# Gardlin/PCR-CG

Measured on AMD Instinct MI355X. Metric: fragment-pairs/s KPFCNN+GCN fwd, 30k-pt pairs, higher is better.
Workload: dtype f32

## Files before the change

### include/pcrcg.h

```cpp
#ifndef PCRCG_H
#define PCRCG_H

#include <stddef.h>
#include <stdint.h>

#ifdef __cplusplus
extern "C" {
#endif

#define PCRCG_OK 0
#define PCRCG_EBADARG (-1)
#define PCRCG_EWORKSPACE (-2)
#define PCRCG_ELAUNCH (-3)
#define PCRCG_ECAPACITY (-4)

#define PCRCG_KPOINTS 15

const char* pcrcg_last_error(void);
#define PCRCG_ABI_VERSION 4
int pcrcg_abi_version(void);

int pcrcg_debug_set(const char* spec);
int pcrcg_debug_release(void);

// ... 47 lines not shown
    int forest_ns, forest_nb;
} pcrcg_reorder_job;
size_t pcrcg_kdforest_ws_bytes(int ns, int nb);
int pcrcg_kdforest_build(const float* sup, int ns, const int* slen, int nb, void* forest, size_t forest_bytes,
                         void* stream);
int pcrcg_radius_reorder(const float* q, int nq, const int* qlen, int nbq, const float* sup, int ns, int nb,
                         const void* forest, int cloud0, float radius, const int* rows, int nrows, const int* count,
                         int max_count, int cols, int64_t* idx, int* status, void* stream);
int pcrcg_radius_reorder_jobs(const pcrcg_reorder_job* jobs, int njobs, const float* sup, int ns, int nb,
                              const void* forest, int* status, void* stream);

size_t pcrcg_kpconv_ws_bytes(int ns);
int pcrcg_kpconv_aggregate(const float* q_pts, int nq, const float* s_pts, int ns, const int64_t* idx,
                           int h, int ld_idx, const float* x, int cin, const float* kp, float extent,
                           float* wf, float* inv_n, void* ws, size_t ws_bytes, void* stream);
int pcrcg_kpconv_c1_layer(const float* q_pts, int nq, const float* s_pts, int ns, const int64_t* idx, int h, int ld_idx,
                          const float* x, const float* kp, float extent, const float* wt, int cout, float* out, int ld_out,
                          float* inv_n, void* sums, void* ws, size_t ws_bytes, void* stream);
int pcrcg_kpconv_aggregate_bf16(const float* q_pts, int nq, const float* s_pts, int ns, const int64_t* idx, int h,
                                int ld_idx, const float* x, int cin, const float* kp, float extent, void* x_bf16,
                                void* wf_bf16, float* inv_n, void* ws, size_t ws_bytes, void* stream);

int pcrcg_kpconv_aggregate_ex(const float* q_pts, int nq, const float* s_pts, int ns, const int64_t* idx, int h,
                              int ld_idx, const float* x, int cin, const float* kp, float extent,
                              const float* offset_features, int ld_off, int influence, int closest, int modulated,
                              float* wf, float* inv_n, float* min_d2, void* ws, size_t ws_bytes, void* stream);

int pcrcg_query_walk(const float* points, int n, int* walk, int* key, void* stream);
int pcrcg_kpconv_aggregate_walk(const float* q_pts, int nq, const float* s_pts, int ns, const int64_t* idx,
                                int h, int ld_idx, const float* x, int cin, const float* kp, float extent,
                                float* wf, float* inv_n, void* ws, size_t ws_bytes, const int* walk, void* stream);
int pcrcg_kpconv_aggregate_bf16_walk(const float* q_pts, int nq, const float* s_pts, int ns, const int64_t* idx, int h,
                                     int ld_idx, const float* x, int cin, const float* kp, float extent, void* x_bf16,
                                     void* wf_bf16, float* inv_n, void* ws, size_t ws_bytes, const int* walk, void* stream);
int pcrcg_gather_max_walk(const float* x, int ns, int c, const int64_t* idx, int nq, int h, int ld_idx,
                          float* out, const int* walk, void* stream);

void pcrcg_profile_kpconv(int enable);
int pcrcg_profile_kpconv_read(float* ms, int* nq, int* h, int* cin, int* cout, int* kind, int cap);

int pcrcg_gemm_f32(const float* a, int lda, const float* b, int ldb, int trans_b, float* c, int ldc, int m,
                   int n, int k, const float* row_scale, const float* bias, void* stream);
size_t pcrcg_gemm_colstats_bytes(int m, int n);
int pcrcg_gemm_f32_colstats(const float* a, int lda, const float* b, int ldb, int trans_b, float* c, int ldc,
                            int m, int n, int k, const float* row_scale, const float* bias, void* colstats,
                            size_t colstats_bytes, int* h_chunks, void* stream);
int pcrcg_gemm_bf16a_f32_colstats(const void* a_bf16, int lda, const float* b, int ldb, float* c, int ldc, int m, int n,
                                  int k, const float* row_scale, const float* bias, void* colstats,
                                  size_t colstats_bytes, int* h_chunks, void* stream);

int pcrcg_gemm_f32_fused(const float* a, int lda, const int64_t* idx, int ld_idx, int ns, const float* zero_row,
                         const void* a_sums, double a_count, float a_eps, float a_slope, const float* b, int ldb,
                         const float* bias, float* c, int ldc, int m, int n, int k, int accumulate, void* stream);

void pcrcg_gemm_set_mode(int mode);
int pcrcg_gemm_get_mode(void);
int pcrcg_gemm_redo_counts(unsigned long long* out2, int reset);
void pcrcg_thread_shares_gpu(int on);

int pcrcg_gather_max(const float* x, int ns, int c, const int64_t* idx, int nq, int h, int ld_idx,
                     float* out, void* stream);
int pcrcg_gather_first(const float* x, int ns, int c, const int64_t* idx, int nq, int ld_idx, float* out,
                       int ld_out, void* stream);
int pcrcg_gather_first_multi(const float* const* x, const int* ns, const int64_t* const* idx, const int* nq, const int* ld_idx,
                             float* const* out, int count, int c, int ld_x, int ld_out, void* stream);
size_t pcrcg_instnorm_ws_bytes(int c);
int pcrcg_instnorm_stats_from_partials(const void* partials, int chunks, int c, double count, float eps,
                                       float* stats, void* stream);
int pcrcg_instnorm_stats(const float* x, int n, int c, int ldx, float eps, float* stats, void* ws,
                         size_t ws_bytes, void* stream);
int pcrcg_instnorm_apply(const float* x, int n, int c, int ldx, const float* stats, const float* res,
                         int ldr, const float* res_stats, float slope, float* y, int ldy, void* stream);
int pcrcg_instnorm_colsums(const float* x, int n, int c, int ldx, void* sums, void* stream);
int pcrcg_instnorm_apply_sums(const float* x, int n, int c, int ldx, const void* sums, double count, float eps,
                              const float* res, int ldr, const void* res_sums, float slope, float* y, int ldy,
                              void* stream);

int pcrcg_fill2d(float* dst, int ld, int rows, int cols, float value, void* stream);
int pcrcg_inject_image_features(const float* fmap, int c, int h, int w, const float* valid, const int64_t* inds2d,
                                const int64_t* inds3d, int n, long row_offset, long n_rows, float* x, int ldx,
                                void* stream);

typedef struct pcrcg_image_frame {
    const float* fmap;
    const float* depth;
    const float* valid;
    float world2camera[16];
    float intrinsics[16];
    float thresh;
    int h, w;
    int depth_h, depth_w;
    int target;
} pcrcg_image_frame;

size_t pcrcg_project_depth_ws_bytes(int n);
int pcrcg_project_depth(const float* points, int n, const float* depth, int h, int w, const float* h_world2camera,
                        const float* h_intrinsics, float thresh, int64_t* inds2d, int64_t* inds3d, int* k, void* ws,
                        size_t ws_bytes, void* stream);
int pcrcg_inject_frames(const float* points, long n_points, long len_src, const pcrcg_image_frame* h_frames, int n_frames,
                        int c, float* x, int ldx, void* stream);
int pcrcg_superglue_valid_maps(const float* keypoints0, int n0, const float* keypoints1, int n1, const int64_t* matches,
                               const float* confidence, int window, int map_w, int map_h, float* src_valid, float* tgt_valid,
                               void* stream);

int pcrcg_knn(const float* coords, int n, int k, int* idx, void* stream);
size_t pcrcg_edgeconv_ws_bytes(int c);
int pcrcg_edgeconv_reduce(const float* ctr, int ld_ctr, const float* nbr, int ld_nbr, const int* idx,
                          int n, int k, int c, float eps, float* emax, int ld_emax, float* stats,
                          void* ws, size_t ws_bytes, void* stream);
int pcrcg_edgeconv_reduce_sums(const float* ctr, int ld_ctr, const float* nbr, int ld_nbr, const int* idx, int n, int k,
                               int c, float* emax, int ld_emax, void* sums, void* stream);
int pcrcg_softmax_rows(float* x, int rows, int cols, int ld, float scale, void* stream);
int pcrcg_attention_supported(int d);
int pcrcg_attention(const float* q, int ldq, const float* k, int ldk, const float* v, int ldv, float* out, int ldo, int n,
                    int ms, int heads, int d, float scale, void* stream);
int pcrcg_softmax_matvec(const float* x, int rows, int cols, int ld, float scale, const float* vec, int ldv, float* y,
                         int ldy, void* stream);

// ... 202 lines not shown
```

### pcrcg_amd/_lib.py

```python
import ctypes
import os

_HERE = os.path.dirname(os.path.abspath(__file__))
LIB_PATH = os.path.join(_HERE, "libpcrcg_hip.so")


def lib_identity():
    import hashlib
    with open(LIB_PATH, "rb") as f:
        return LIB_PATH, hashlib.sha256(f.read()).hexdigest()[:16]

ABI_VERSION = 4

c_int, c_float, c_void_p, c_size_t = ctypes.c_int, ctypes.c_float, ctypes.c_void_p, ctypes.c_size_t

SIGNATURES = {
    "pcrcg_last_error": (ctypes.c_char_p, []),
    "pcrcg_abi_version": (c_int, []),
    "pcrcg_debug_set": (c_int, [ctypes.c_char_p]),
    "pcrcg_check_status": (c_int, [c_void_p, c_void_p]),
    "pcrcg_grid_subsample_ws_bytes": (c_size_t, [c_int, c_int]),
    "pcrcg_grid_subsample_batch": (c_int, [c_void_p, c_int, c_void_p, c_int, c_float, c_int, c_void_p, c_void_p,
                                           c_void_p, c_void_p, c_size_t, c_void_p]),
    "pcrcg_grid_subsample_ex_ws_bytes": (c_size_t, [c_int, c_int, c_int, c_int]),
    "pcrcg_grid_subsample_batch_ex": (c_int, [c_void_p, c_int, c_void_p, c_int, c_float, c_int, c_void_p, c_int, c_int,
                                              c_void_p, c_int, c_void_p, c_void_p, c_void_p, c_void_p, c_void_p, c_void_p,
                                              c_size_t, c_void_p]),
    "pcrcg_umap_order_ws_bytes": (c_size_t, [c_int]),
    "pcrcg_umap_order": (c_int, [c_void_p, c_int, c_void_p, c_void_p, c_size_t, c_void_p]),
    "pcrcg_cellgrid_ws_bytes": (c_size_t, [c_int, c_int]),
    "pcrcg_cellgrid_build": (c_int, [c_void_p, c_int, c_void_p, c_int, c_float, c_void_p, c_size_t, c_void_p]),
    "pcrcg_radius_query": (c_int, [c_void_p, c_int, c_void_p, c_int, c_void_p, c_int, c_float, c_void_p, c_int,
                                   c_void_p, c_void_p, c_void_p, c_void_p, c_void_p]),
    "pcrcg_radius_query_ex": (c_int, [c_void_p, c_int, c_void_p, c_int, c_void_p, c_int, c_float, c_void_p, c_int,
                                      c_void_p, c_void_p, c_void_p, c_void_p, c_void_p, c_void_p, c_void_p]),
    "pcrcg_radius_query_groups": (c_int, [c_void_p, c_int, c_void_p, c_int, c_void_p, c_int, c_int, c_float, c_void_p, c_int,
                                          c_void_p, c_void_p, c_void_p, c_void_p, c_void_p, c_void_p, c_void_p]),
    "pcrcg_radius_query_cells": (c_int, [c_void_p, c_void_p, c_int, c_void_p, c_void_p, c_int, c_void_p, c_int, c_int, c_float,
                                         c_int, c_void_p, c_void_p, c_void_p, c_void_p, c_void_p, c_void_p, c_void_p]),
    "pcrcg_kdforest_ws_bytes": (c_size_t, [c_int, c_int]),
    "pcrcg_kdforest_build": (c_int, [c_void_p, c_int, c_void_p, c_int, c_void_p, c_size_t, c_void_p]),
    "pcrcg_radius_reorder": (c_int, [c_void_p, c_int, c_void_p, c_int, c_void_p, c_int, c_int, c_void_p, c_int,
                                     c_float, c_void_p, c_int, c_void_p, c_int, c_int, c_void_p, c_void_p, c_void_p]),
    "pcrcg_radius_reorder_jobs": (c_int, [c_void_p, c_int, c_void_p, c_int, c_int, c_void_p, c_void_p, c_void_p]),
    "pcrcg_radius_neighbors_ws_bytes": (c_size_t, [c_int, c_int]),
    "pcrcg_radius_neighbors_batch": (c_int, [c_void_p, c_int, c_void_p, c_int, c_void_p, c_void_p, c_int, c_float,
                                             c_int, c_void_p, c_void_p, c_void_p, c_void_p, c_void_p, c_size_t,
                                             c_void_p]),
    "pcrcg_kpconv_ws_bytes": (c_size_t, [c_int]),
    "pcrcg_kpconv_aggregate": (c_int, [c_void_p, c_int, c_void_p, c_int, c_void_p, c_int, c_int, c_void_p, c_int,
                                       c_void_p, c_float, c_void_p, c_void_p, c_void_p, c_size_t, c_void_p]),
    "pcrcg_kpconv_c1_layer": (c_int, [c_void_p, c_int, c_void_p, c_int, c_void_p, c_int, c_int, c_void_p, c_void_p, c_float,
                                      c_void_p, c_int, c_void_p, c_int, c_void_p, c_void_p, c_void_p, c_size_t, c_void_p]),
    "pcrcg_kpconv_aggregate_bf16": (c_int, [c_void_p, c_int, c_void_p, c_int, c_void_p, c_int, c_int, c_void_p, c_int,
                                            c_void_p, c_float, c_void_p, c_void_p, c_void_p, c_void_p, c_size_t,
                                            c_void_p]),
    "pcrcg_kpconv_aggregate_ex": (c_int, [c_void_p, c_int, c_void_p, c_int, c_void_p, c_int, c_int, c_void_p, c_int,
                                          c_void_p, c_float, c_void_p, c_int, c_int, c_int, c_int, c_void_p, c_void_p,
                                          c_void_p, c_void_p, c_size_t, c_void_p]),
    "pcrcg_query_walk": (c_int, [c_void_p, c_int, c_void_p, c_void_p, c_void_p]),
    "pcrcg_kpconv_aggregate_walk": (c_int, [c_void_p, c_int, c_void_p, c_int, c_void_p, c_int, c_int, c_void_p, c_int,
                                            c_void_p, c_float, c_void_p, c_void_p, c_void_p, c_size_t, c_void_p, c_void_p]),
    "pcrcg_kpconv_aggregate_bf16_walk": (c_int, [c_void_p, c_int, c_void_p, c_int, c_void_p, c_int, c_int, c_void_p, c_int,
                                                 c_void_p, c_float, c_void_p, c_void_p, c_void_p, c_void_p, c_size_t,
                                                 c_void_p, c_void_p]),
    "pcrcg_gather_max_walk": (c_int, [c_void_p, c_int, c_int, c_void_p, c_int, c_int, c_int, c_void_p, c_void_p, c_void_p]),
    "pcrcg_profile_kpconv": (None, [c_int]),
    "pcrcg_profile_kpconv_read": (c_int, [c_void_p, c_void_p, c_void_p, c_void_p, c_void_p, c_void_p, c_int]),
    "pcrcg_gemm_f32": (c_int, [c_void_p, c_int, c_void_p, c_int, c_int, c_void_p, c_int, c_int, c_int, c_int,
                               c_void_p, c_void_p, c_void_p]),
    "pcrcg_gemm_colstats_bytes": (c_size_t, [c_int, c_int]),
    "pcrcg_gemm_f32_colstats": (c_int, [c_void_p, c_int, c_void_p, c_int, c_int, c_void_p, c_int, c_int, c_int, c_int,
                                        c_void_p, c_void_p, c_void_p, c_size_t, c_void_p, c_void_p]),
    "pcrcg_gemm_bf16a_f32_colstats": (c_int, [c_void_p, c_int, c_void_p, c_int, c_void_p, c_int, c_int, c_int, c_int,
                                              c_void_p, c_void_p, c_void_p, c_size_t, c_void_p, c_void_p]),
    "pcrcg_gemm_f32_fused": (c_int, [c_void_p, c_int, c_void_p, c_int, c_int, c_void_p, c_void_p, ctypes.c_double, c_float,
                                     c_float, c_void_p, c_int, c_void_p, c_void_p, c_int, c_int, c_int, c_int, c_int, c_void_p]),
    "pcrcg_gemm_set_mode": (None, [c_int]),
    "pcrcg_gemm_get_mode": (c_int, []),
    "pcrcg_gemm_redo_counts": (c_int, [c_void_p, c_int]),
    "pcrcg_instnorm_stats_from_partials": (c_int, [c_void_p, c_int, c_int, ctypes.c_double, c_float, c_void_p,
                                                   c_void_p]),
    "pcrcg_gather_max": (c_int, [c_void_p, c_int, c_int, c_void_p, c_int, c_int, c_int, c_void_p, c_void_p]),
    "pcrcg_gather_first": (c_int, [c_void_p, c_int, c_int, c_void_p, c_int, c_int, c_void_p, c_int, c_void_p]),
    "pcrcg_gather_first_multi": (c_int, [c_void_p, c_void_p, c_void_p, c_void_p, c_void_p, c_void_p, c_int, c_int, c_int, c_int,
                                         c_void_p]),
    "pcrcg_instnorm_ws_bytes": (c_size_t, [c_int]),
    "pcrcg_instnorm_stats": (c_int, [c_void_p, c_int, c_int, c_int, c_float, c_void_p, c_void_p, c_size_t, c_void_p]),
    "pcrcg_instnorm_apply": (c_int, [c_void_p, c_int, c_int, c_int, c_void_p, c_void_p, c_int, c_void_p, c_float,
                                     c_void_p, c_int, c_void_p]),
    "pcrcg_instnorm_colsums": (c_int, [c_void_p, c_int, c_int, c_int, c_void_p, c_void_p]),
    "pcrcg_instnorm_apply_sums": (c_int, [c_void_p, c_int, c_int, c_int, c_void_p, ctypes.c_double, c_float, c_void_p, c_int,
                                          c_void_p, c_float, c_void_p, c_int, c_void_p]),
    "pcrcg_fill2d": (c_int, [c_void_p, c_int, c_int, c_int, c_float, c_void_p]),
    "pcrcg_inject_image_features": (c_int, [c_void_p, c_int, c_int, c_int, c_void_p, c_void_p, c_void_p, c_int, ctypes.c_long,
                                            ctypes.c_long, c_void_p, c_int, c_void_p]),
    "pcrcg_project_depth_ws_bytes": (c_size_t, [c_int]),
    "pcrcg_project_depth": (c_int, [c_void_p, c_int, c_void_p, c_int, c_int, c_void_p, c_void_p, c_float, c_void_p, c_void_p,
                                    c_void_p, c_void_p, c_size_t, c_void_p]),
    "pcrcg_inject_frames": (c_int, [c_void_p, ctypes.c_long, ctypes.c_long, c_void_p, c_int, c_int, c_void_p, c_int, c_void_p]),
    "pcrcg_superglue_valid_maps": (c_int, [c_void_p, c_int, c_void_p, c_int, c_void_p, c_void_p, c_int, c_int, c_int, c_void_p,
                                           c_void_p, c_void_p]),
    "pcrcg_knn": (c_int, [c_void_p, c_int, c_int, c_void_p, c_void_p]),
    "pcrcg_edgeconv_ws_bytes": (c_size_t, [c_int]),
    "pcrcg_edgeconv_reduce": (c_int, [c_void_p, c_int, c_void_p, c_int, c_void_p, c_int, c_int, c_int, c_float,
                                      c_void_p, c_int, c_void_p, c_void_p, c_size_t, c_void_p]),
    "pcrcg_edgeconv_reduce_sums": (c_int, [c_void_p, c_int, c_void_p, c_int, c_void_p, c_int, c_int, c_int, c_void_p, c_int,
                                           c_void_p, c_void_p]),
    "pcrcg_softmax_rows": (c_int, [c_void_p, c_int, c_int, c_int, c_float, c_void_p]),
    "pcrcg_attention_supported": (c_int, [c_int]),
    "pcrcg_attention": (c_int, [c_void_p, c_int, c_void_p, c_int, c_void_p, c_int, c_void_p, c_int, c_int, c_int, c_int,
                                c_int, c_float, c_void_p]),
    "pcrcg_softmax_matvec": (c_int, [c_void_p, c_int, c_int, c_int, c_float, c_void_p, c_int, c_void_p, c_int, c_void_p]),
    "pcrcg_copy2d": (c_int, [c_void_p, c_int, c_void_p, c_int, c_int, c_int, c_void_p]),
    "pcrcg_add": (c_int, [c_void_p, c_void_p, c_void_p, ctypes.c_long, c_void_p]),
    "pcrcg_l2norm_rows": (c_int, [c_void_p, c_int, c_void_p, c_int, c_int, c_int, c_void_p]),
    "pcrcg_sigmoid_scores": (c_int, [c_void_p, c_int, c_void_p, c_int, c_void_p]),
    "pcrcg_kpfcnn_ws_bytes": (c_size_t, [c_void_p, c_void_p]),
    "pcrcg_kpfcnn_group_ws_bytes": (c_size_t, [c_void_p, c_void_p, c_int]),
    "pcrcg_kpfcnn_forward_group": (c_int, [c_void_p, c_void_p, c_void_p, c_int, c_void_p, c_size_t, c_void_p]),
    "pcrcg_kpfcnn_forward": (c_int, [c_void_p, c_void_p, c_void_p, c_void_p, c_size_t, c_void_p]),
    "pcrcg_pyramid_ws_bytes": (c_size_t, [c_int, c_int, c_void_p]),
    "pcrcg_pyramid_build": (c_int, [c_void_p, c_int, c_void_p, c_int, c_void_p, c_void_p, c_size_t, c_void_p, c_void_p,
                                    c_void_p, c_void_p, c_void_p, c_void_p]),
    "pcrcg_pyramid_build_parts": (c_int, [c_void_p, c_void_p, c_void_p, c_void_p, c_int, c_void_p, c_void_p, c_size_t, c_void_p,
                                          c_void_p, c_void_p, c_void_p, c_void_p, c_void_p]),
    "pcrcg_pyramid_restore_run": (c_int, [c_void_p, c_void_p, c_void_p]),
    "pcrcg_debug_release": (c_int, []),
    "pcrcg_stream_pipe_classes": (c_int, [c_void_p, c_int, c_void_p, c_void_p]),
    "pcrcg_thread_shares_gpu": (None, [c_int]),
    "pcrcg_stream_create": (c_int, [c_void_p, c_int]),
    "pcrcg_stream_destroy": (c_int, [c_void_p]),
    "pcrcg_ransac_ws_bytes": (c_size_t, [c_int, c_int, c_int, c_int]),
    "pcrcg_feature_match": (c_int, [c_void_p, c_int, c_int, c_void_p, c_int, c_int, c_int, c_int, c_void_p, c_void_p,
                                    c_void_p, c_size_t, c_void_p]),
    "pcrcg_ransac": (c_int, [c_void_p, c_int, c_void_p, c_int, c_void_p, c_void_p, c_int, c_void_p, c_int, ctypes.c_double,
                             ctypes.c_double, c_int, c_int, c_int, ctypes.c_uint64, c_void_p, c_void_p, c_void_p, c_void_p,
# ... 141 lines not shown
```

### pcrcg_amd/csrc/common.h

```cpp
#pragma once
#include <hip/hip_runtime.h>

#include <cstdarg>
#include <cstdint>
#include <cstdio>
#include <map>
#include <mutex>

#include "pcrcg.h"

namespace pcrcg {

void set_error(const char* fmt, ...);

inline hipStream_t as_stream(void* s) { return reinterpret_cast<hipStream_t>(s); }

struct Carver {
    char* base;
    size_t cap;
    size_t off = 0;
    Carver(void* ws, size_t bytes) : base(static_cast<char*>(ws)), cap(bytes) {}
    template <typename T>
    T* take(size_t count) {
        size_t bytes = (count * sizeof(T) + 255) & ~size_t(255);
// ... 10 lines not shown

constexpr int kWave = 64;

bool instnorm_pack_ok(int c, int ldx, int ldy);
int instnorm_apply_pack(const float* x, int n, int c, int ldx, const float* stats, const double* sums, double count, float eps,
                        float slope, float* y, int ldy, const float* s_pts, float4* pk, hipStream_t st);
size_t colstats_ws_bytes(int c);
int colstats_finalize(const double* partial, int nchunks, int c, double count, float eps, float* stats,
                      hipStream_t st);
int colstats_chunks();
float4* kpconv_pk_ptr(void* ws, size_t ws_bytes, int ns);

class StreamScratch {
public:
    explicit StreamScratch(bool cleared = false);
    void* get(hipStream_t st, size_t bytes, size_t slack = 0);
    void release();
private:
    struct Buf { void* p = nullptr; size_t bytes = 0; };
    const bool cleared_;
    std::mutex mu_;
    std::map<hipStream_t, Buf> bufs_;
};

int kpconv_pack(const float* x, int ns, int cin, const float* s_pts, void* ws, size_t ws_bytes, hipStream_t st,
                unsigned short* x_bf16 = nullptr);
int kpconv_aggregate_rows(const float* q_pts, int nq, const float* s_pts, int ns, const int64_t* idx, int h, int ld_idx,
                          const float* x, int cin, const float* kp, float extent, float* wf, float* inv_n, void* ws,
                          size_t ws_bytes, hipStream_t st, bool pack, bool stream_out, int c1_ld = 0,
                          const int* walk = nullptr);
bool kpconv_c1_fused_ok(int cout, const float* wt);
int kpconv_c1_fused(const float* q_pts, int nq, const float* s_pts, int ns, const int64_t* idx, int h, int ld_idx, const float* x,
                    const float* kp, float extent, const float* wt, int cout, float* y, int ld_y, float* inv_n, double* sums,
                    void* ws, size_t ws_bytes, hipStream_t st, bool pack);
int kpconv_aggregate_bf16(const float* q_pts, int nq, const float* s_pts, int ns, const int64_t* idx, int h, int ld_idx,
                          const float* x, unsigned short* x_bf16, int cin, const float* kp, float extent,
                          unsigned short* wf_bf16, float* inv_n, void* ws, size_t ws_bytes, hipStream_t st,
                          const int* walk = nullptr);

int query_walk_multi(const float* const* pts, const int* n, int* const* walk, int* const* key, int count, hipStream_t st);

struct NormJob {
    const float* x; const double* sums; const float* res; const double* res_sums; float* y;
    const float* s_pts; float4* pk;
    int n; double count;
    float* stats_out = nullptr;
};
int instnorm_apply_sums_multi(const NormJob* jobs, int count, int c, int ldx, float eps, int ldr, float slope, int ldy, bool pack,
                              hipStream_t st);
bool instnorm_sums_ok(int c, int ldx, int ldy, int ldr = 0);

struct GatherJob { const float* x; const int64_t* idx; float* out; int ns, nq, h, ld_idx; const int* walk = nullptr; };
int gather_max_multi(const GatherJob* jobs, int count, int c, hipStream_t st);
struct FirstJob { const float* x; const int64_t* idx; float* out; int ns, nq, ld_idx; };
int gather_first_multi(const FirstJob* jobs, int count, int c, int ld_x, int ld_out, hipStream_t st);
int heads_multi(const float* const* x, const int* rows, int count, int ld, int fd, float* const* feats, float* const* s_ov,
                float* const* s_sal, hipStream_t st);
int copy2d_multi(const float* const* src, float* const* dst, const int* rows, int count, int ld_src, int ld_dst, int cols,
                 hipStream_t st);
int instnorm_colsums_multi(const float* const* x, double* const* sums, const int* n, int count, int c, int ldx, hipStream_t st);

struct EdgeCloud {
    const float* ctr; const float* nbr; const int* idx; float* emax; double* sums; int n, k;
};
bool edgeconv_rows_ok(const EdgeCloud* cl, int count, int ld_ctr, int ld_nbr, int ld_emax, int c);
int edgeconv_rows_multi(const EdgeCloud* cl, int count, int ld_ctr, int ld_nbr, int ld_emax, int c, bool atomic, int* nchunks_out,
                        hipStream_t st);

struct AttnCloud { const float* q; const float* k; const float* v; float* out; int n, ms; };
bool attention_mfma_ok(const AttnCloud* cl, int count, int ldq, int ldk, int ldv, int d);
int attention_mfma_multi(const AttnCloud* cl, int count, int ldq, int ldk, int ldv, int ldo, int heads, int d, float scale,
                         hipStream_t st);
bool attention_bwd_mfma_ok(int n, int ms, int d, int ldq, int ldk, int ldv, int ld_do);
int attention_bwd_mfma(const float* q, int ldq, const float* k, int ldk, const float* v, int ldv, const float* o, int ldo,
                       const float* d_o, int ld_do, float* dq, int ld_dq, float* dk, int ld_dk, float* dv, int ld_dv, int n, int ms,
                       int heads, int d, float scale, hipStream_t st);

struct DebugOpts {
    int stat_sums = 1;
    int stat_sums_rows = 1 << 30;
    int att_mfma = 1;
    int radius_blocks = 0;
    int kd_blocks = 0;
    int att_tq = 16;
    int kd_spin_limit = 0;
    int gemm_log = 0;
    int x6_tile = -1, x6_splitk = 0, x6_t1 = 1, x6_t2 = 1, x6_order = -1, x6_big = 0, x6_h2 = 1;
    int train_side_stream = 1;
    int gemm_tile = -1, gemm_splitk = 0, gemm_split_target = 768;
    int deterministic = 0;
    int bwd_mfma = 1;
    int walk = 1;
};
const DebugOpts& debug_opts();

struct KpProfScope {
    hipStream_t st;
    hipEvent_t a, b;
    int nq, h, cin, cout, kind;
    bool on;
    KpProfScope(hipStream_t s, int nq, int h, int cin, int cout, int kind);
    ~KpProfScope();
};

}

#define PCRCG_CHECK_ARG(cond)                                                        \
    do {                                                                             \
        if (!(cond)) {                                                               \
            pcrcg::set_error("%s: bad argument: %s", __func__, #cond);               \
            return PCRCG_EBADARG;                                                    \
        }                                                                            \
    } while (0)

#define PCRCG_CHECK_WS(carver)                                                                     \
    do {                                                                                           \
        if (!(carver).ok()) {                                                                      \
            pcrcg::set_error("%s: workspace too small (%zu needed, %zu given)", __func__,          \
                             (carver).off, (carver).cap);                                          \
            return PCRCG_EWORKSPACE;                                                               \
        }                                                                                          \
    } while (0)

#define PCRCG_CHECK_HIP(expr)                                                                  \
    do {                                                                                       \
        hipError_t e_ = (expr);                                                                \
        if (e_ != hipSuccess) {                                                                \
            pcrcg::set_error("%s: %s failed: %s", __func__, #expr, hipGetErrorString(e_));     \
            return PCRCG_ELAUNCH;                                                              \
        }                                                                                      \
    } while (0)

#define PCRCG_CHECK_LAUNCH() PCRCG_CHECK_HIP(hipGetLastError())

namespace pcrcg {
inline hipError_t grant_max_dyn_lds(const void* kern) {
    hipFuncAttributes at;
    hipError_t e = hipFuncGetAttributes(&at, kern);
    if (e != hipSuccess) return e;
    const int cap = 160 * 1024 - (int)at.sharedSizeBytes;
    return hipFuncSetAttribute(kern, hipFuncAttributeMaxDynamicSharedMemorySize, cap);
}
}
#define PCRCG_GRANT_LDS(kern)                                                                                   \
    do {                                                                                                        \
// ... 12 lines not shown
```

### pcrcg_amd/csrc/gemm.h

```cpp
#pragma once
#include "common.h"

namespace pcrcg {

struct GemmExtra {
    const long long* a_idx = nullptr;
    int a_idx_ld = 0, a_ns = 0;
    const float* a_zero = nullptr;
    bool accumulate = false;
    const double* a_sums = nullptr;
    double a_count = 0.0;
    float a_eps = 1e-5f, a_slope = 1.0f;
    int grad_operand = 0;
};

struct GemmPair {
    const float* a = nullptr;
    float* c = nullptr;
    int m = 0;
    const float* row_scale = nullptr;
    void* colstats = nullptr;
    int* h_chunks = nullptr;
    bool c_zeroed = false;
    const long long* a_idx = nullptr;
    int a_ns = 0;
    const double* a_sums = nullptr;
    double a_count = 0.0;
};
struct GemmGroup {
    int n = 0;
    GemmPair p[3];
};

enum class GemmA { row_f32, kmajor_f32, row_bf16 };
enum class GemmB { nk, kn };

struct GemmCall {
    const void* a = nullptr;
    const float* b = nullptr;
    float* c = nullptr;
    int lda = 0, ldb = 0, ldc = 0;
    int m = 0, n = 0, k = 0;
    GemmA a_form = GemmA::row_f32;
    GemmB b_form = GemmB::nk;
    const float* row_scale = nullptr;
    const float* bias = nullptr;
    void* colstats = nullptr;
    size_t colstats_bytes = 0;
    int* h_chunks = nullptr;
    bool colstats_sums = false;
    bool c_zeroed = false;
    const GemmExtra* ex = nullptr;
    const GemmGroup* grp = nullptr;
    hipStream_t st = nullptr;
};

int gemm_run(const GemmCall& g);
bool gemm_split_terms_on();
bool gemm_bt_accumulates(int m, int n, int k, long m_total = 0);

int gemm_x6_dispatch(const GemmCall& g);
int gemm_x6_splits(int m, int n, int k, long m_total);
int gemm_x6_redo_counts(unsigned long long* out, int reset);
bool gemm_x6_shared();
void gemm_x6_set_shared(int on);

}
```

### pcrcg_amd/csrc/gemm.hip

```cpp
#include <cstdlib>

#include <atomic>

#include "gemm.h"
#include "pcrcg_train.h"

namespace pcrcg {
namespace {

typedef float f32x16 __attribute__((ext_vector_type(16)));
template <int BM, int BN, bool TRANS_A, bool TRANS_B, int BK>
constexpr int stage_floats() {
    return (TRANS_A ? BK * (BM + 4) : BM * (BK + 4)) + (TRANS_B ? BN * (BK + 4) : BK * (BN + 4));
}

template <int BM, int BN, int WAVES_M, int WAVES_N, bool TRANS_A, bool TRANS_B, int BK>
__global__ void __launch_bounds__(256) k_gemm_f32(const float* __restrict__ A, int lda, const float* __restrict__ B,
                                                   int ldb, float* __restrict__ C, int ldc, int M, int N, int Kdim,
                                                   const float* __restrict__ row_scale, const float* __restrict__ bias,
                                                   int k_per_split, int vec_a, int vec_b, int atomic_out,
                                                   double* __restrict__ colp, int colp_chunks) {
    static_assert(WAVES_M * WAVES_N == 4, "4 wavefronts per block");
    constexpr int WM = BM / WAVES_M, WN = BN / WAVES_N;
    constexpr int TM = WM / 32, TN = WN / 32;
// ... 302 lines not shown
        return (long)((m + tiles[t].bm - 1) / tiles[t].bm) * ((n + tiles[t].bn - 1) / tiles[t].bn);
    };
    int pick = debug_opts().gemm_tile;
    if (pick < 0 || pick > 3) pick = (n > 64 && ntiles(0) >= 1024) ? 0 : 3;
    if (trans_a) pick = 3;
    const int BM = tiles[pick].bm, BN = tiles[pick].bn;
    const int gx = (n + BN - 1) / BN, gy = (m + BM - 1) / BM;
    int splits = 1;
    const int ktiles = (k + BK - 1) / BK;
    const int split_target = debug_opts().gemm_split_target;
    const int max_splits = trans_a ? 256 : 32;
    while ((long)gx * gy * splits < split_target && k / (2 * splits) >= 192 && splits < max_splits) splits *= 2;
    if (debug_opts().gemm_splitk > 0) splits = debug_opts().gemm_splitk;
    p.k_per_split = ((ktiles + splits - 1) / splits) * BK;
    if (p.k_per_split < BK) p.k_per_split = BK;
    splits = k > 0 ? (k + p.k_per_split - 1) / p.k_per_split : 1;
    if (splits < 1) splits = 1;
    p.atomic_out = splits > 1;
    if (p.atomic_out) {
        if (g.ldc == n) PCRCG_CHECK_HIP(hipMemsetAsync(g.c, 0, (size_t)m * n * sizeof(float), g.st));
        else PCRCG_CHECK_HIP(hipMemset2DAsync(g.c, (size_t)g.ldc * sizeof(float), 0, (size_t)n * sizeof(float), m, g.st));
    }
    const dim3 grid(gx, gy, splits);
    const bool want_partials = g.colstats && g.h_chunks && !g.colstats_sums;
    if (debug_opts().gemm_log != 0)
        fprintf(stderr, "pcrcg_gemm m=%d n=%d k=%d lda=%d ldb=%d ldc=%d tb=%d grid=%dx%dx%d rs=%d bias=%d stats=%d\n", m, n, k,
                g.lda, g.ldb, g.ldc, (int)trans_b, gx, gy, splits, g.row_scale != nullptr, g.bias != nullptr,
                g.colstats != nullptr && !g.colstats_sums);
    if (want_partials && !p.atomic_out) {
        const int chunks = gy * (pick == 1 ? 4 : 2);
        if (carve_bytes(2 * (size_t)n * chunks, sizeof(double)) <= g.colstats_bytes) {
            p.colp = static_cast<double*>(g.colstats);
            p.colp_chunks = *g.h_chunks = chunks;
        }
    }
    if (trans_a)
        return trans_b ? launch_f32<64, 64, 2, 2, true, true>(p, grid, g.st) : launch_f32<64, 64, 2, 2, true, false>(p, grid, g.st);
    if (pick == 0) return launch_f32_tile<128, 128, 2, 2>(trans_b, p, grid, g.st);
    if (pick == 1) return launch_f32_tile<128, 64, 4, 1>(trans_b, p, grid, g.st);
    if (pick == 2) return launch_f32_tile<64, 128, 2, 2>(trans_b, p, grid, g.st);
    return launch_f32_tile<64, 64, 2, 2>(trans_b, p, grid, g.st);
}

}

bool gemm_split_terms_on() { return gemm_mode() == 1; }

bool gemm_bt_accumulates(int m, int n, int k, long m_total) { return gemm_split_terms_on() && gemm_x6_splits(m, n, k, m_total) > 1; }

int gemm_run(const GemmCall& g) {
    if (g.h_chunks) *g.h_chunks = 0;
    const bool trans_a = g.a_form == GemmA::kmajor_f32, b_kn = g.b_form == GemmB::kn, bf16 = g.a_form == GemmA::row_bf16;
    const bool grouped = g.grp && g.grp->n != 0;
    const bool x6_form = g.ex || grouped || bf16;
    PCRCG_CHECK_ARG(g.m >= 0 && g.n >= 0 && g.k >= 0);
    const bool ld_ok = (trans_a ? g.lda >= g.m : g.lda >= g.k) && (b_kn ? g.ldb >= g.n : g.ldb >= g.k) && g.ldc >= g.n;
    if (x6_form) PCRCG_CHECK_ARG(g.k >= 1 && ld_ok && !(trans_a && !b_kn));
    if (grouped) PCRCG_CHECK_ARG(g.m >= 1 && g.n >= 1);
    if (bf16) PCRCG_CHECK_ARG(g.k % 32 == 0 && g.lda % 8 == 0);
    if (g.m == 0 || g.n == 0) return PCRCG_OK;
    PCRCG_CHECK_ARG(g.a && g.b && g.c);
    PCRCG_CHECK_ARG(ld_ok);
    if (bf16) {
        PCRCG_CHECK_ARG((reinterpret_cast<uintptr_t>(g.a) & 15) == 0 && g.ldb % 4 == 0 && (reinterpret_cast<uintptr_t>(g.b) & 15) == 0);
        return gemm_x6_dispatch(g);
    }
    if (x6_form) PCRCG_CHECK_ARG(gemm_split_terms_on());
    if (gemm_split_terms_on() && !(trans_a && !b_kn)) return gemm_x6_dispatch(g);
    return gemm_f32_dispatch(g);
}

}

using namespace pcrcg;

extern "C" void pcrcg_gemm_set_mode(int mode) { g_gemm_mode.store(mode != 0, std::memory_order_relaxed); }
extern "C" int pcrcg_gemm_get_mode(void) { return gemm_mode(); }
extern "C" void pcrcg_thread_shares_gpu(int on) { gemm_x6_set_shared(on); }
extern "C" int pcrcg_gemm_redo_counts(unsigned long long* out2, int reset) { return gemm_x6_redo_counts(out2, reset); }

extern "C" size_t pcrcg_gemm_colstats_bytes(int m, int n) {
    const size_t chunks = (size_t)((m > 0 ? m : 1) + 31) / 32 + 4;
    return carve_bytes(2 * (size_t)(n > 0 ? n : 1) * chunks, sizeof(double));
}

static GemmCall plain_call(const void* a, int lda, int trans_a, const float* b, int ldb, int trans_b, float* c, int ldc, int m,
                           int n, int k, const float* row_scale, const float* bias, void* stream) {
    GemmCall g;
    g.a = a; g.lda = lda; g.b = b; g.ldb = ldb; g.c = c; g.ldc = ldc;
    g.m = m; g.n = n; g.k = k;
    g.a_form = trans_a ? GemmA::kmajor_f32 : GemmA::row_f32;
    g.b_form = trans_b ? GemmB::nk : GemmB::kn;
    g.row_scale = row_scale; g.bias = bias;
    g.st = as_stream(stream);
    return g;
}

extern "C" int pcrcg_gemm_f32(const float* a, int lda, const float* b, int ldb, int trans_b, float* c, int ldc,
                              int m, int n, int k, const float* row_scale, const float* bias, void* stream) {
    return gemm_run(plain_call(a, lda, 0, b, ldb, trans_b, c, ldc, m, n, k, row_scale, bias, stream));
}

extern "C" int pcrcg_gemm_f32_colstats(const float* a, int lda, const float* b, int ldb, int trans_b, float* c,
                                       int ldc, int m, int n, int k, const float* row_scale, const float* bias,
                                       void* colstats, size_t colstats_bytes, int* h_chunks, void* stream) {
    GemmCall g = plain_call(a, lda, 0, b, ldb, trans_b, c, ldc, m, n, k, row_scale, bias, stream);
    g.colstats = colstats; g.colstats_bytes = colstats_bytes; g.h_chunks = h_chunks;
    return gemm_run(g);
}

extern "C" int pcrcg_gemm_bf16a_f32_colstats(const void* a_bf16, int lda, const float* b, int ldb, float* c, int ldc, int m,
                                             int n, int k, const float* row_scale, const float* bias, void* colstats,
                                             size_t colstats_bytes, int* h_chunks, void* stream) {
    GemmCall g = plain_call(a_bf16, lda, 0, b, ldb, 1, c, ldc, m, n, k, row_scale, bias, stream);
    g.a_form = GemmA::row_bf16;
    g.colstats = colstats; g.colstats_bytes = colstats_bytes; g.h_chunks = h_chunks;
    return gemm_run(g);
}

extern "C" int pcrcg_gemm_f32_fused(const float* a, int lda, const int64_t* idx, int ld_idx, int ns, const float* zero_row,
                                    const void* a_sums, double a_count, float a_eps, float a_slope, const float* b, int ldb,
                                    const float* bias, float* c, int ldc, int m, int n, int k, int accumulate, void* stream) {
    PCRCG_CHECK_ARG(!idx || (ld_idx >= 1 && ns >= 0 && zero_row));
    PCRCG_CHECK_ARG(!a_sums || a_count >= 1.0);
    if (!gemm_split_terms_on()) {
        set_error("pcrcg_gemm_f32_fused: only the split-bf16 arithmetic (pcrcg_gemm_set_mode(1)) implements it");
        return PCRCG_EBADARG;
    }
    GemmExtra ex;
    ex.a_idx = reinterpret_cast<const long long*>(idx);
    ex.a_idx_ld = ld_idx;
    ex.a_ns = ns;
    ex.a_zero = zero_row;
    ex.accumulate = accumulate != 0;
    ex.a_sums = static_cast<const double*>(a_sums);
    ex.a_count = a_count;
    ex.a_eps = a_eps;
    ex.a_slope = a_slope;
    GemmCall g = plain_call(a, lda, 0, b, ldb, 1, c, ldc, m, n, k, nullptr, bias, stream);
    g.ex = &ex;
    return gemm_run(g);
}

extern "C" int pcrcg_gemm_f32_ex(const float* a, int lda, int trans_a, const float* b, int ldb, int trans_b, float* c,
                                 int ldc, int m, int n, int k, const float* row_scale, const float* bias, void* stream) {
    return gemm_run(plain_call(a, lda, trans_a, b, ldb, trans_b, c, ldc, m, n, k, row_scale, bias, stream));
}

extern "C" int pcrcg_gemm_f32_grad(const float* a, int lda, int trans_a, const float* b, int ldb, int trans_b, float* c,
                                   int ldc, int m, int n, int k, const float* row_scale, const float* bias, int grad_operand,
                                   void* stream) {
    PCRCG_CHECK_ARG(grad_operand >= 0 && grad_operand <= 2);
    GemmCall g = plain_call(a, lda, trans_a, b, ldb, trans_b, c, ldc, m, n, k, row_scale, bias, stream);
    if (grad_operand == 0 || !gemm_split_terms_on() || (trans_a && trans_b)) return gemm_run(g);
    PCRCG_CHECK_ARG(m >= 0 && n >= 0 && k >= 0);
    if (m == 0 || n == 0 || k == 0) return PCRCG_OK;
    GemmExtra ex;
    ex.grad_operand = grad_operand;
    g.ex = &ex;
    return gemm_run(g);
}
```

### pcrcg_amd/csrc/gemm_x6.hip

```cpp
#include <cstdlib>
#include <type_traits>

#include <hip/hip_ext.h>

#include "gemm.h"
#include "pcrcg_train.h"

namespace pcrcg {
namespace {

typedef float f32x16 __attribute__((ext_vector_type(16)));
typedef __bf16 bf16x8 __attribute__((ext_vector_type(8)));
typedef unsigned int u32x4 __attribute__((ext_vector_type(4)));

typedef float f32x4 __attribute__((ext_vector_type(4)));
typedef float f32x2 __attribute__((ext_vector_type(2)));
typedef _Float16 f16x2 __attribute__((ext_vector_type(2)));
typedef _Float16 f16x8 __attribute__((ext_vector_type(8)));

constexpr int BK = 32;

__device__ unsigned long long g_x6_redo[2];

constexpr int kGroupExtra = 3;
struct GemmPairArgs {
    int extra = 0;
    int off[kGroupExtra] = {0, 0, 0}, m[kGroupExtra] = {0, 0, 0};
    const float* a[kGroupExtra] = {nullptr, nullptr, nullptr};
    float* c[kGroupExtra] = {nullptr, nullptr, nullptr};
    const float* rs[kGroupExtra] = {nullptr, nullptr, nullptr};
    double* colp[kGroupExtra] = {nullptr, nullptr, nullptr};
    int colp_chunks[kGroupExtra] = {0, 0, 0};
    const long long* a_idx[kGroupExtra] = {nullptr, nullptr, nullptr};
    int a_ns[kGroupExtra] = {0, 0, 0};
    const double* a_sums[kGroupExtra] = {nullptr, nullptr, nullptr};
    double a_count[kGroupExtra] = {0.0, 0.0, 0.0};
};

__device__ __forceinline__ void gload16(f32x4& dst, const float* p) {
    asm volatile("global_load_dwordx4 %0, %1, off" : "=v"(dst) : "v"(p) : "memory");
}
template <int N>
__device__ __forceinline__ void vm_wait() {
    asm volatile("s_waitcnt vmcnt(%0)" ::"n"(N) : "memory");
}
__device__ __forceinline__ void pin(f32x4& r) { asm volatile("" : "+v"(r)); }
__device__ __forceinline__ void gload4(float& dst, const float* p) {
    asm volatile("global_load_dword %0, %1, off" : "=v"(dst) : "v"(p) : "memory");
}
__device__ __forceinline__ void pin(float& r) { asm volatile("" : "+v"(r)); }

template <int LAY> struct Item;
template <> struct Item<0> {
    f32x4 v[2];
    static constexpr int LOADS = 2;
    __device__ __forceinline__ float get(int i) const { return v[i >> 2][i & 3]; }
    __device__ __forceinline__ void set(int i, float x) { v[i >> 2][i & 3] = x; }
    __device__ __forceinline__ void hold() { pin(v[0]); pin(v[1]); }
};
template <> struct Item<1> {
    float s[8];
    static constexpr int LOADS = 8;
    __device__ __forceinline__ float get(int i) const { return s[i]; }
    __device__ __forceinline__ void set(int i, float x) { s[i] = x; }
    __device__ __forceinline__ void hold() {
#pragma unroll
        for (int i = 0; i < 8; ++i) pin(s[i]);
    }
};
template <int LAY, int ROWS>
__device__ __forceinline__ void item_pos(int e, int& row, int& kg) {
    if (LAY == 0) { row = e >> 2; kg = e & 3; }
    else { row = e % ROWS; kg = e / ROWS; }
}
template <int LAY, int ROWS>
__device__ __forceinline__ void item_load_fast(Item<LAY>& d, const float* __restrict__ P, int ld, int row0, int rows, int k0,
                                               int e) {
    int row, kg;
    item_pos<LAY, ROWS>(e, row, kg);
    if constexpr (LAY == 0) {
        const float* p = P + (long)min(row0 + row, rows - 1) * ld + k0 + kg * 8;
        gload16(d.v[0], p);
        gload16(d.v[1], p + 4);
    } else {
        const float* p = P + (long)(k0 + kg * 8) * ld + min(row0 + row, rows - 1);
#pragma unroll
        for (int j = 0; j < 8; ++j) gload4(d.s[j], p + (long)j * ld);
    }
}
template <int LAY, int ROWS>
__device__ __forceinline__ void item_load_edge(Item<LAY>& d, const float* __restrict__ P, int ld, int row0, int rows, int k0,
                                               int k_end, int e) {
    int row, kg;
    item_pos<LAY, ROWS>(e, row, kg);
    const int gr = row0 + row, gk = k0 + kg * 8, ke = k_end - 1;
    const bool rok = gr < rows;
    float v[8];
#pragma unroll
    for (int j = 0; j < 8; ++j)
        v[j] = LAY == 0 ? P[(long)min(gr, rows - 1) * ld + min(gk + j, ke)] : P[(long)min(gk + j, ke) * ld + min(gr, rows - 1)];
#pragma unroll
    for (int j = 0; j < 8; ++j) d.set(j, (rok && gk + j < k_end) ? v[j] : 0.f);
}

#include "split_terms.h"

template <int BM, int BN>
constexpr int lds_bytes() { return 3 * (BM + BN) * ROWB; }
template <int BM, int BN>
constexpr int x6_threads() { return (BM == 128 && BN == 128) ? 512 : 256; }

struct TileMap { int gx, gy, gs, order; long split_stride; };
static int x6_tile_order(int gx, int gy, int gs, int bm, int bn, int k_per_split) {
    const int forced = debug_opts().x6_order;
    if (forced >= 0 && forced <= 2) return forced;
    const double a_blk = 4.0 * bm * k_per_split, b_blk = 4.0 * bn * k_per_split, keep = 2.0e6;
    const double total = (double)gx * gy * gs, q = total / 8.0;
    const double per_split = (double)gx * gy;
    const double splits_touched = q >= per_split ? q / per_split : 1.0;
    const double in_split = q >= per_split ? per_split : q;
    double rows0 = in_split / gx; if (rows0 < 1.0) rows0 = 1.0;
    const double cols0 = in_split < gx ? in_split : gx;
    const double b0 = cols0 * b_blk, a0 = rows0 * a_blk;
    const double cost0 = splits_touched * (a0 + (b0 <= keep ? b0 : b0 * rows0));
    double cols1 = in_split / gy; if (cols1 < 1.0) cols1 = 1.0;
    const double rows1 = in_split < gy ? in_split : gy;
    const double a1 = rows1 * a_blk, b1 = cols1 * b_blk;
    const double cost1 = splits_touched * (b1 + (a1 <= keep ? a1 : a1 * cols1));
    return cost1 < 0.9 * cost0 ? 1 : 0;
}

template <int BM, int BN, int MINB, int ATERMS, int ALAY, int BLAY, int ANORM = 0, int KNOCK = 0, int H2 = 0>
__global__ void __launch_bounds__((x6_threads<BM, BN>()), MINB) k_gemm_x6(const float* __restrict__ A, int lda, const float* __restrict__ B,
                                                        int ldb, float* __restrict__ C, int ldc, int M, int N, int Kdim,
                                                        const float* __restrict__ row_scale,
                                                        const float* __restrict__ bias, int k_per_split, int vec_a,
                                                        int vec_b, int atomic_out, double* __restrict__ colp,
                                                        int colp_chunks, const long long* __restrict__ a_idx,
                                                        int a_idx_ld, int a_ns, const float* __restrict__ a_zero,
                                                        const double* __restrict__ a_sums, double a_count, float a_eps,
                                                        float a_slope, GemmPairArgs pr, TileMap tm, float h2_sa, float h2_sb) {
    constexpr int NT = x6_threads<BM, BN>();
    constexpr int WAVES_M = 2, WAVES_N = NT / 128;
    constexpr int WM = BM / WAVES_M, WN = BN / WAVES_N;
    constexpr int TM = WM / 32, TN = WN / 32;
    constexpr int A_ITERS = BM * 4 / NT;
    constexpr int B_ITERS = BN * 4 / NT;
    constexpr int A_PLANE = BM * ROWB, B_PLANE = BN * ROWB;
    static_assert(A_ITERS >= 1 && B_ITERS >= 1, "tile too small");
    extern __shared__ __attribute__((aligned(16))) unsigned char smem[];
    unsigned char* const As = smem;
    unsigned char* const Bs = smem + 3 * A_PLANE;

    const int tid = threadIdx.x, lane = tid & 63, wave = __builtin_amdgcn_readfirstlane((int)(threadIdx.x >> 6));
    const int wm = wave / WAVES_N, wn = wave % WAVES_N;
    const int gx = tm.gx;
    int ntile = tm.gx * tm.gy * tm.gs, lin = blockIdx.x, base = 0;
    if (tm.order == 2) {
        ntile = tm.gx * tm.gy;
        base = lin / ntile * ntile;
        lin -= base;
    }
    const int xq = ntile >> 3, xr = ntile & 7, xcd = lin & 7, slot = lin >> 3;
    const int tile = base + (xcd < xr ? xcd * (xq + 1) : xr * (xq + 1) + (xcd - xr) * xq) + slot;
    int tile_x, tile_y;
    const int split = tile / (tm.gx * tm.gy), in_split = tile % (tm.gx * tm.gy);
    if (tm.order != 1) {
        tile_x = in_split % gx;
        tile_y = in_split / gx;
    } else {
        tile_y = in_split % tm.gy;
        tile_x = in_split / tm.gy;
    }
    int m0 = tile_y * BM;
    const int n0 = tile_x * BN;
    if (pr.extra > 0 && m0 >= pr.off[0]) {
        int e = 0;
        if (pr.extra > 1 && m0 >= pr.off[1]) e = 1;
        if (pr.extra > 2 && m0 >= pr.off[2]) e = 2;
        m0 -= pr.off[e];
        tile_y = m0 / BM;
        M = pr.m[e];
        A = pr.a[e];
        C = pr.c[e];
        row_scale = pr.rs[e];
        colp = pr.colp[e];
        colp_chunks = pr.colp_chunks[e];
        a_idx = pr.a_idx[e];
        a_ns = pr.a_ns[e];
        a_sums = pr.a_sums[e];
        a_count = pr.a_count[e];
    }
    const int k_begin = split * k_per_split;
    const int k_end = min(Kdim, k_begin + k_per_split);
    C += (long)split * tm.split_stride;

    f32x16 acc[TM][TN];
    f32x16 acc_lo[H2 ? TM : 1][H2 ? TN : 1];
#pragma unroll
    for (int i = 0; i < TM; ++i)
#pragma unroll
        for (int j = 0; j < TN; ++j)
#pragma unroll
            for (int r = 0; r < 16; ++r) {
                acc[i][j][r] = 0.0f;
                if constexpr (H2) acc_lo[i][j][r] = 0.0f;
            }

    const float* arow[A_ITERS];
    bool arok[A_ITERS], azero[A_ITERS];
    if constexpr (ALAY == 0 && ATERMS == 3) {
#pragma unroll
        for (int it = 0; it < A_ITERS; ++it) {
            const int gr = m0 + ((tid + it * NT) >> 2);
            const int r = min(gr, M - 1);
            arok[it] = gr < M;
            azero[it] = false;
            if (a_idx) {
                const long long g = a_idx[(long)r * a_idx_ld];
                azero[it] = !(g >= 0 && g < a_ns);
                arow[it] = azero[it] ? a_zero : A + g * lda;
            } else {
                arow[it] = A + (long)r * lda;
            }
        }
    }
    float* const s_mean = reinterpret_cast<float*>(smem + 3 * (A_PLANE + B_PLANE));
    float* const s_rstd = s_mean + (ANORM ? ((k_per_split + BK - 1) / BK) * BK : 0);
    int* const s_ovf = reinterpret_cast<int*>(s_rstd + (ANORM ? ((k_per_split + BK - 1) / BK) * BK : 0));
    unsigned* const s_seen = reinterpret_cast<unsigned*>(As + 2 * A_PLANE);
    static_assert(!H2 || (BM + BN) * 4 <= A_PLANE, "row words must fit the unused plane");
    if constexpr (H2) {
        if (tid == 0) *s_ovf = 0;
        for (int i = tid; i < BM + BN; i += NT) s_seen[i] = 0u;
        if constexpr (!ANORM) __syncthreads();
    }
    if constexpr (ANORM) {
        for (int kk = tid; kk < k_end - k_begin; kk += NT) {
            const double mu = a_sums[k_begin + kk] / a_count;
            double var = a_sums[(long)Kdim + k_begin + kk] / a_count - mu * mu;
            if (var < 0.0) var = 0.0;
            s_mean[kk] = (float)mu;
            s_rstd[kk] = (float)(1.0 / sqrt(var + (double)a_eps));
        }
// ... 458 lines not shown
        __syncthreads();
#pragma unroll
        for (int j = 0; j < TN; ++j) {
            const double s = ds[j] + __shfl_xor(ds[j], 32, 64), q2 = dq[j] + __shfl_xor(dq[j], 32, 64);
            const int gn = n0 + wn * WN + j * 32 + l31;
            if (wm == 0 && half == 0 && gn < N) {
                unsafeAtomicAdd(&colp[gn], s + red[2 * (wn * WN + j * 32 + l31)]);
                unsafeAtomicAdd(&colp[(long)N + gn], q2 + red[2 * (wn * WN + j * 32 + l31) + 1]);
            }
        }
    } else if (colp) {
        const int chunk = tile_y * WAVES_M + wm;
#pragma unroll
        for (int j = 0; j < TN; ++j) {
            const double s = ds[j] + __shfl_xor(ds[j], 32, 64), q2 = dq[j] + __shfl_xor(dq[j], 32, 64);
            const int gn = n0 + wn * WN + j * 32 + l31;
            if (half == 0 && gn < N) {
                colp[(long)gn * colp_chunks + chunk] = s;
                colp[((long)N + gn) * colp_chunks + chunk] = q2;
            }
        }
    }
}

StreamScratch g_splitk_partials;

__global__ void __launch_bounds__(256) k_split_reduce(const float* __restrict__ part, long stride, int splits, float* __restrict__ c,
                                                      int ldc, int m, int n, int accumulate) {
    const long t = (long)blockIdx.x * 256 + threadIdx.x;
    if (t >= (long)m * n) return;
    const long r = t / n;
    const int col = (int)(t - r * n);
    float sum = part[t];
    for (int s = 1; s < splits; ++s) sum += part[(long)s * stride + t];
    float* dst = c + r * ldc + col;
    *dst = accumulate ? *dst + sum : sum;
}

struct X6Args {
    const float* a; int lda;
    const float* b; int ldb;
    float* c; int ldc;
    int m, n, k;
    const float* row_scale; const float* bias;
    int k_per_split, vec_a, vec_b, atomic_out;
    double* colp = nullptr; int colp_chunks = 0;
    const long long* a_idx = nullptr; int a_idx_ld = 0, a_ns = 0;
    const float* a_zero = nullptr;
    const double* a_sums = nullptr; double a_count = 0.0;
    float a_eps = 0.f, a_slope = 1.f;
    GemmPairArgs pr;
    long split_stride = 0;
    float h2_sa = 1.f, h2_sb = 1.f;
};

template <int BM, int BN, int MINB, int ATERMS, int ALAY, int BLAY, int ANORM = 0, int KNOCK = 0, int H2 = 0>
int launch_x6(const X6Args& p, dim3 grid, hipStream_t st) {
    TileMap tm;
    tm.split_stride = p.split_stride;
    tm.gx = (int)grid.x;
    tm.gy = (int)grid.y;
    tm.gs = (int)grid.z;
    tm.order = x6_tile_order(tm.gx, tm.gy, tm.gs, BM, BN, p.k_per_split);
    const size_t lds = lds_bytes<BM, BN>() + (ANORM ? 2 * sizeof(float) * (size_t)(((p.k_per_split + BK - 1) / BK) * BK) : 0) + (H2 ? 16 : 0);
    auto kern = k_gemm_x6<BM, BN, MINB, ATERMS, ALAY, BLAY, ANORM, KNOCK, H2>;
    PCRCG_GRANT_LDS(kern);
    int m_all = p.m;
    for (int e = 0; e < p.pr.extra; ++e) m_all += p.pr.m[e];
    KpProfScope prof(st, m_all, p.n, p.k, (ATERMS == 1 || H2) ? 3 : 6, 3);
    hipExtLaunchKernelGGL(kern, dim3(tm.gx * tm.gy * tm.gs), dim3(x6_threads<BM, BN>()), lds, st, prof.a, prof.b, 0, p.a, p.lda, p.b,
                          p.ldb, p.c, p.ldc, p.m, p.n, p.k, p.row_scale, p.bias, p.k_per_split, p.vec_a, p.vec_b, p.atomic_out,
                          p.colp, p.colp_chunks, p.a_idx, p.a_idx_ld, p.a_ns, p.a_zero, p.a_sums, p.a_count, p.a_eps, p.a_slope,
                          p.pr, tm, p.h2_sa, p.h2_sb);
    PCRCG_CHECK_LAUNCH();
    return PCRCG_OK;
}
template <int BM, int BN, int MINB>
int launch_x6_abt(bool h2, bool a_bf16, const X6Args& p, dim3 grid, hipStream_t st) {
    if (h2) return launch_x6<BM, BN, MINB, 3, 0, 0, 0, 0, 1>(p, grid, st);
    if (a_bf16) return launch_x6<BM, BN, MINB, 1, 0, 0>(p, grid, st);
    return launch_x6<BM, BN, MINB, 3, 0, 0>(p, grid, st);
}

}

static thread_local int g_x6_shared = 0;
bool gemm_x6_shared() { return g_x6_shared > 0; }
void gemm_x6_set_shared(int on) { g_x6_shared = on ? 1 : 0; }

struct X6Plan { int pick, bm, bn, gx, gy, splits, k_per_split; };
static X6Plan x6_plan_for(int pick, int m, int n, int k, bool reduce_rows) {
    static const int tiles[4][2] = {{128, 128}, {128, 64}, {64, 128}, {64, 64}};
    X6Plan p;
    p.pick = pick;
    p.bm = tiles[p.pick][0];
    p.bn = tiles[p.pick][1];
    p.gx = (n + p.bn - 1) / p.bn;
    p.gy = (m + p.bm - 1) / p.bm;
    int splits = 1;
    const int ktiles = (k + BK - 1) / BK;
    const int max_splits = reduce_rows ? 128 : 32;
    int t1 = 200, t2 = 1024;
    if (gemm_x6_shared() && !reduce_rows) { t1 = debug_opts().x6_t1; t2 = debug_opts().x6_t2; }
    while ((long)p.gx * p.gy * splits < t1 && k / (2 * splits) >= 256 && splits < max_splits) splits *= 2;
    while ((long)p.gx * p.gy * splits < t2 && k / splits > 1024 && splits < max_splits) splits *= 2;
    if (debug_opts().x6_splitk > 0) splits = debug_opts().x6_splitk;
    p.k_per_split = ((ktiles + splits - 1) / splits) * BK;
    if (p.k_per_split < BK) p.k_per_split = BK;
    p.splits = k > 0 ? (k + p.k_per_split - 1) / p.k_per_split : 1;
    if (p.splits < 1) p.splits = 1;
    return p;
}
static X6Plan x6_plan(int m, int n, int k, bool kmajor = false, bool reduce_rows = false, long m_total = 0) {
    int pick = debug_opts().x6_tile;
    if (kmajor) return x6_plan_for(3, m, n, k, reduce_rows);
    if (pick >= 0 && pick <= 3) return x6_plan_for(pick, m, n, k, reduce_rows);
    if (n >= 128 && debug_opts().x6_big) {
        const X6Plan big = x6_plan_for(0, m, n, k, reduce_rows);
        const long rows = m_total > m ? m_total : m;
        if ((long)big.gx * ((rows + 127) / 128) * big.splits >= 240) return big;
    }
    return x6_plan_for((n <= 64 && m >= 32768) ? 1 : 3, m, n, k, reduce_rows);
}

int gemm_x6_redo_counts(unsigned long long* out, int reset) {
    if (out) PCRCG_CHECK_HIP(hipMemcpyFromSymbol(out, HIP_SYMBOL(g_x6_redo), sizeof(unsigned long long) * 2));
    if (reset) {
        const unsigned long long z[2] = {0ull, 0ull};
        PCRCG_CHECK_HIP(hipMemcpyToSymbol(HIP_SYMBOL(g_x6_redo), z, sizeof(z)));
    }
    return PCRCG_OK;
}

int gemm_x6_splits(int m, int n, int k, long m_total) { return (m > 0 && n > 0) ? x6_plan(m, n, k, false, false, m_total).splits : 1; }

static int x6_run(const GemmCall& g, long split_stride) {
    const float* const a = static_cast<const float*>(g.a);
    const int m = g.m, n = g.n, k = g.k, ldc = g.ldc;
    const bool a_bf16 = g.a_form == GemmA::row_bf16, a_kmajor = g.a_form == GemmA::kmajor_f32, b_kmajor = g.b_form == GemmB::kn;
    const GemmExtra* const ex = g.ex;
    const GemmGroup* const grp = g.grp;
    hipStream_t st = g.st;
    if (a_kmajor && !b_kmajor) { set_error("gemm_x6: A^T * B^T is not built"); return PCRCG_EBADARG; }
    int m_plan = m;
    const int n_extra = grp ? grp->n : 0;
    if (n_extra < 0 || n_extra > kGroupExtra) { set_error("gemm_x6: at most %d further products per launch", kGroupExtra); return PCRCG_EBADARG; }
    for (int e = 0; e < n_extra; ++e) {
        if (grp->p[e].m <= 0 || !grp->p[e].a || !grp->p[e].c) { set_error("gemm_x6: empty product in a group"); return PCRCG_EBADARG; }
        m_plan = grp->p[e].m > m_plan ? grp->p[e].m : m_plan;
    }
    long m_total = m;
    for (int e = 0; e < n_extra; ++e) m_total += grp->p[e].m;
    const bool accumulate = ex && ex->accumulate;
    const bool gather = ex && ex->a_idx;
    const bool anorm = ex && ex->a_sums;
    const int grad_op = ex ? ex->grad_operand : 0;
    const bool h2 = debug_opts().x6_h2 != 0 && !a_bf16;
    const bool lifted = h2 && grad_op;
    const X6Plan plan = x6_plan(m_plan, n, k, a_kmajor || b_kmajor || anorm || lifted, a_kmajor, m_total);
    const int BM = plan.bm, gx = plan.gx, splits = plan.splits;
    const int gy0 = (m + BM - 1) / BM;
    int gy = gy0, gye[kGroupExtra] = {0, 0, 0};
    for (int e = 0; e < n_extra; ++e) { gye[e] = (grp->p[e].m + BM - 1) / BM; gy += gye[e]; }
    if (n_extra && (a_kmajor || b_kmajor)) { set_error("gemm_x6: grouped launches are built for the A * B^T form"); return PCRCG_EBADARG; }
    if ((gather && (a_bf16 || a_kmajor || b_kmajor)) || (accumulate && a_bf16)) {
        set_error("gemm_x6: gather is built for k-contiguous fp32 operands, accumulate for fp32 operands");
        return PCRCG_EBADARG;
    }
    if (gather && !ex->a_zero) { set_error("gemm_x6: gather needs a zero row"); return PCRCG_EBADARG; }
    if (anorm && (a_bf16 || a_kmajor || b_kmajor || plan.pick != 3)) {
        set_error("gemm_x6: normalise-on-load is built for the 64 x 64 tile of k-contiguous fp32 operands");
        return PCRCG_EBADARG;
    }
    if (splits > 1 && debug_opts().deterministic && !split_stride) {
        const size_t floats = (size_t)splits * (size_t)m_total * (size_t)n;
        float* part = static_cast<float*>(g_splitk_partials.get(st, floats * sizeof(float), (floats / 4) * sizeof(float)));
        if (!part) { set_error("gemm_x6: no memory for the deterministic mode's partial tiles"); return PCRCG_ELAUNCH; }
        GemmCall g2 = g;
        g2.c = part;
        g2.ldc = n;
        g2.colstats = nullptr;
        g2.colstats_bytes = 0;
        g2.h_chunks = nullptr;
        g2.colstats_sums = false;
        g2.c_zeroed = true;
        GemmExtra ex2;
        if (ex) { ex2 = *ex; ex2.accumulate = false; g2.ex = &ex2; }
        GemmGroup grp2;
        size_t row = (size_t)m;
        if (grp) {
            grp2 = *grp;
            for (int e = 0; e < n_extra; ++e) {
                grp2.p[e].c = part + row * (size_t)n;
                grp2.p[e].c_zeroed = true;
                grp2.p[e].colstats = nullptr;
                if (grp->p[e].h_chunks) *grp->p[e].h_chunks = 0;
                grp2.p[e].h_chunks = nullptr;
                row += (size_t)grp->p[e].m;
            }
            g2.grp = &grp2;
        }
        const long stride = (long)((size_t)m_total * (size_t)n);
        PCRCG_PROPAGATE(x6_run(g2, stride));
        row = 0;
        for (int e = -1; e < n_extra; ++e) {
            const int me = e < 0 ? m : grp->p[e].m;
            float* ce = e < 0 ? g.c : grp->p[e].c;
            const long total = (long)me * n;
            hipLaunchKernelGGL(k_split_reduce, dim3((unsigned)((total + 255) / 256)), dim3(256), 0, st, part + row * (size_t)n,
                               stride, splits, ce, ldc, me, n, accumulate ? 1 : 0);
            row += (size_t)me;
        }
        PCRCG_CHECK_LAUNCH();
        return PCRCG_OK;
    }
    X6Args p{a, g.lda, g.b, g.ldb, g.c, ldc, m, n, k, g.row_scale, g.bias, plan.k_per_split};
    p.vec_a = (a_bf16 || a_kmajor) ? 1 : (g.lda % 4 == 0) && ((reinterpret_cast<uintptr_t>(a) & 15) == 0);
    p.vec_b = b_kmajor ? 1 : (g.ldb % 4 == 0) && ((reinterpret_cast<uintptr_t>(g.b) & 15) == 0);
    p.split_stride = split_stride;
    p.atomic_out = split_stride ? 0 : (splits > 1 || accumulate);
    for (int e = -1; e < n_extra; ++e) {
        float* ce = e < 0 ? g.c : grp->p[e].c;
        const int me = e < 0 ? m : grp->p[e].m;
        if (splits > 1 && !(e < 0 ? g.c_zeroed : grp->p[e].c_zeroed) && !accumulate) {
            if (ldc == n) PCRCG_CHECK_HIP(hipMemsetAsync(ce, 0, (size_t)me * n * sizeof(float), st));
            else PCRCG_CHECK_HIP(hipMemset2DAsync(ce, (size_t)ldc * sizeof(float), 0, (size_t)n * sizeof(float), me, st));
        }
    }
    const dim3 grid(gx, gy, splits);
    if (debug_opts().gemm_log != 0)
        fprintf(stderr, "pcrcg_gemm_x6 m=%d n=%d k=%d lda=%d ldb=%d ldc=%d tile=%dx%d grid=%dx%dx%d rs=%d bias=%d stats=%d\n", m,
                n, k, g.lda, g.ldb, ldc, BM, plan.bn, gx, gy, splits, g.row_scale != nullptr, g.bias != nullptr, g.colstats != nullptr);
    if (g.colstats && g.h_chunks && !p.atomic_out && g.colstats_sums) {
        if (2 * (size_t)n * sizeof(double) <= g.colstats_bytes) {
            p.colp = static_cast<double*>(g.colstats);
            p.colp_chunks = *g.h_chunks = -1;
        }
    } else if (g.colstats && g.h_chunks && !p.atomic_out) {
        const int chunks = gy0 * 2;
        if (carve_bytes(2 * (size_t)n * chunks, sizeof(double)) <= g.colstats_bytes) {
            p.colp = static_cast<double*>(g.colstats);
            p.colp_chunks = *g.h_chunks = chunks;
        }
    }
    GemmPairArgs& pa = p.pr;
    pa.extra = n_extra;
    int row_off = gy0 * BM;
    for (int e = 0; e < n_extra; ++e) {
        const GemmPair& q = grp->p[e];
        pa.off[e] = row_off;
        row_off += gye[e] * BM;
        pa.m[e] = q.m;
        pa.a[e] = q.a;
        pa.c[e] = q.c;
        pa.rs[e] = q.row_scale;
        pa.a_idx[e] = q.a_idx;
        pa.a_ns[e] = q.a_ns;
        pa.a_sums[e] = q.a_sums;
        pa.a_count[e] = q.a_count;
        if (q.h_chunks) *q.h_chunks = 0;
        if (p.colp && q.colstats && q.h_chunks) {
            pa.colp[e] = static_cast<double*>(q.colstats);
            pa.colp_chunks[e] = p.colp_chunks < 0 ? -1 : gye[e] * 2;
            *q.h_chunks = pa.colp_chunks[e];
            if (p.colp_chunks > 0 && carve_bytes(2 * (size_t)n * pa.colp_chunks[e], sizeof(double)) > g.colstats_bytes) {
                pa.colp[e] = nullptr;
                pa.colp_chunks[e] = 0;
                *q.h_chunks = 0;
            }
        }
    }
    if (gather) { p.a_idx = ex->a_idx; p.a_idx_ld = ex->a_idx_ld; p.a_ns = ex->a_ns; p.a_zero = ex->a_zero; }
    if (anorm) { p.a_sums = ex->a_sums; p.a_count = ex->a_count; p.a_eps = ex->a_eps; p.a_slope = ex->a_slope; }
    if (lifted && !anorm) { p.h2_sa = grad_op == 1 ? 65536.0f : 1.0f; p.h2_sb = grad_op == 2 ? 65536.0f : 1.0f; }
    if (a_kmajor)
        return lifted ? launch_x6<64, 64, 3, 3, 1, 1, 0, 0, 2>(p, grid, st) : launch_x6<64, 64, 3, 3, 1, 1>(p, grid, st);
    if (b_kmajor)
        return lifted ? launch_x6<64, 64, 4, 3, 0, 1, 0, 0, 2>(p, grid, st) : launch_x6<64, 64, 4, 3, 0, 1>(p, grid, st);
    if (lifted && !anorm)
        return launch_x6<64, 64, 4, 3, 0, 0, 0, 0, 2>(p, grid, st);
    if (anorm) return h2 ? launch_x6<64, 64, 4, 3, 0, 0, 1, 0, 1>(p, grid, st) : launch_x6<64, 64, 4, 3, 0, 0, 1>(p, grid, st);
    if (plan.pick == 0) return launch_x6_abt<128, 128, 2>(h2, a_bf16, p, grid, st);
    if (plan.pick == 1) return launch_x6_abt<128, 64, 2>(h2, a_bf16, p, grid, st);
    if (plan.pick == 2) return launch_x6_abt<64, 128, 2>(h2, a_bf16, p, grid, st);
    return launch_x6_abt<64, 64, 4>(h2, a_bf16, p, grid, st);
}

int gemm_x6_dispatch(const GemmCall& g) { return x6_run(g, 0); }

}
```

### pcrcg_amd/csrc/pointops.hip

```cpp
#include "common.h"

namespace pcrcg {
namespace {

constexpr int kWavesPerBlock = 4;

struct GatherMulti { const float* x[4]; const long long* idx[4]; float* out[4]; int ns[4], nq[4], h[4], ld_idx[4]; const int* walk[4]; };
template <bool VEC4>
__global__ void __launch_bounds__(kWavesPerBlock * 64) k_gather_max(GatherMulti mm, int c, int nchunk) {
    const int g = blockIdx.y;
    const float* __restrict__ x = mm.x[g];
    const long long* __restrict__ idx = mm.idx[g];
    float* __restrict__ out = mm.out[g];
    const int ns = mm.ns[g], nq = mm.nq[g], h = mm.h[g], ld_idx = mm.ld_idx[g];
    const int lane = threadIdx.x & 63;
    const int* __restrict__ walk = mm.walk[g];
    const int wave = __builtin_amdgcn_readfirstlane((int)(threadIdx.x >> 6));
    long item = (long)blockIdx.x * kWavesPerBlock + wave, items = (long)nq * nchunk;
    int pos0 = 0;
    if (walk) {
        const int xcd = blockIdx.x & 7, slot = blockIdx.x >> 3;
        const int xq = nq >> 3, xr = nq & 7;
        pos0 = xcd < xr ? xcd * (xq + 1) : xr * (xq + 1) + (xcd - xr) * xq;
        item = (long)slot * kWavesPerBlock + wave;
        items = (long)(xq + (xcd < xr ? 1 : 0)) * nchunk;
    }
    if (item >= items) return;
    const int p = (int)(item / nchunk), chunk = (int)(item - (long)p * nchunk);
    int q = p;
    if (walk) {
        q = walk[pos0 + p];
        q = q < 0 ? 0 : (q < nq ? q : nq - 1);
    }
    const long long* row = idx + (long)q * ld_idx;
    if (VEC4) {
        const int cb = chunk * 64 + lane;
        if (cb >= (c >> 2)) return;
        float4 m = make_float4(0.f, 0.f, 0.f, 0.f);
        bool any = false;
#pragma unroll 4
        for (int j = 0; j < h; ++j) {
            const long long i = row[j];
            float4 v = make_float4(0.f, 0.f, 0.f, 0.f);
            if (i >= 0 && i < ns) v = reinterpret_cast<const float4*>(x + i * c)[cb];
            if (!any) { m = v; any = true; }
            else { m.x = fmaxf(m.x, v.x); m.y = fmaxf(m.y, v.y); m.z = fmaxf(m.z, v.z); m.w = fmaxf(m.w, v.w); }
        }
        reinterpret_cast<float4*>(out + (long)q * c)[cb] = m;
    } else {
        const int cc = chunk * 64 + lane;
        if (cc >= c) return;
        float m = 0.f;
        bool any = false;
#pragma unroll 4
        for (int j = 0; j < h; ++j) {
            const long long i = row[j];
            const float v = (i >= 0 && i < ns) ? x[i * c + cc] : 0.f;
            m = any ? fmaxf(m, v) : v;
            any = true;
        }
        out[(long)q * c + cc] = m;
    }
}

__global__ void __launch_bounds__(256) k_gather_first(const float* __restrict__ x, int ns, int c,
                                                       const long long* __restrict__ idx, int nq, int ld_idx,
                                                       float* __restrict__ out, int ld_out) {
    const int lane = threadIdx.x & 63;
    const int q = blockIdx.x * 4 + __builtin_amdgcn_readfirstlane((int)(threadIdx.x >> 6));
    if (q >= nq) return;
    const long long i = idx[(long)q * ld_idx];
    const bool real = i >= 0 && i < ns;
    for (int cc = lane; cc < c; cc += 64) out[(long)q * ld_out + cc] = real ? x[i * c + cc] : 0.f;
}

struct FirstMulti { const float* x[4]; const long long* idx[4]; float* out[4]; int ns[4], nq[4], ld_idx[4]; };
template <bool VEC>
__global__ void __launch_bounds__(256) k_gather_first_multi(FirstMulti mm, int c, int ld_x, int ld_out) {
    const int g = blockIdx.y;
    const int segs = (c + 3) >> 2;
    const long t = (long)blockIdx.x * 256 + threadIdx.x;
    const long q = t / segs;
    if (q >= mm.nq[g]) return;
    const int c0 = (int)(t - q * segs) * 4;
    const long long i = mm.idx[g][q * mm.ld_idx[g]];
    const bool real = i >= 0 && i < mm.ns[g];
    const float* __restrict__ src = mm.x[g] + (real ? i : 0) * ld_x + c0;
    float* __restrict__ dst = mm.out[g] + q * ld_out + c0;
    if (VEC && c0 + 4 <= c) {
        *reinterpret_cast<float4*>(dst) = real ? *reinterpret_cast<const float4*>(src) : make_float4(0.f, 0.f, 0.f, 0.f);
    } else {
        const int n = c - c0 < 4 ? c - c0 : 4;
        for (int k = 0; k < n; ++k) dst[k] = real ? src[k] : 0.f;
    }
}

constexpr int kStatChunks = 128;

struct ColsMulti { const float* x[4]; double* partial[4]; int n[4]; };
template <bool ATOMIC>
__global__ void __launch_bounds__(256) k_colstats_partial(ColsMulti mm, int c, int ldx) {
    const float* __restrict__ x = mm.x[blockIdx.z];
    double* __restrict__ partial = mm.partial[blockIdx.z];
    const int n = mm.n[blockIdx.z];
    __shared__ double s_sum[4][64], s_sq[4][64];
    const int lane = threadIdx.x & 63, rl = threadIdx.x >> 6;
    const int ch = blockIdx.y * 64 + lane;
    const int chunk = blockIdx.x, nchunks = gridDim.x;
    const long rows_per = ((long)n + nchunks - 1) / nchunks;
    const long r0 = chunk * rows_per, r1 = min((long)n, r0 + rows_per);
    double s = 0.0, sq = 0.0;
    if (ch < c) {
        long r = r0 + rl;
        for (; r + 12 < r1; r += 16) {
            const float v0 = x[r * ldx + ch], v1 = x[(r + 4) * ldx + ch], v2 = x[(r + 8) * ldx + ch],
                        v3 = x[(r + 12) * ldx + ch];
            s += ((double)v0 + (double)v1) + ((double)v2 + (double)v3);
            sq += ((double)v0 * v0 + (double)v1 * v1) + ((double)v2 * v2 + (double)v3 * v3);
        }
        for (; r < r1; r += 4) {
            const double v = (double)x[r * ldx + ch];
            s += v;
            sq += v * v;
        }
    }
    s_sum[rl][lane] = s;
    s_sq[rl][lane] = sq;
    __syncthreads();
    if (rl == 0 && ch < c) {
        s = (s_sum[0][lane] + s_sum[1][lane]) + (s_sum[2][lane] + s_sum[3][lane]);
        sq = (s_sq[0][lane] + s_sq[1][lane]) + (s_sq[2][lane] + s_sq[3][lane]);
        if (ATOMIC) {
            if (r0 < r1) {
                unsafeAtomicAdd(&partial[ch], s);
                unsafeAtomicAdd(&partial[(long)c + ch], sq);
            }
        } else {
            partial[(long)ch * nchunks + chunk] = s;
            partial[((long)c + ch) * nchunks + chunk] = sq;
        }
// ... 249 lines not shown
        hipLaunchKernelGGL(k_instnorm_apply4_sums_pack, grid, dim3(256), 0, st, mm, c4, ldx, eps, slope, ldy, rows_per_block);
    else if (!jobs[0].res)
        hipLaunchKernelGGL(k_instnorm_apply4_sums<0>, grid, dim3(256), 0, st, mm, c4, ldx, eps, ldr, slope, ldy, rows_per_block);
    else if (!jobs[0].res_sums)
        hipLaunchKernelGGL(k_instnorm_apply4_sums<1>, grid, dim3(256), 0, st, mm, c4, ldx, eps, ldr, slope, ldy, rows_per_block);
    else
        hipLaunchKernelGGL(k_instnorm_apply4_sums<2>, grid, dim3(256), 0, st, mm, c4, ldx, eps, ldr, slope, ldy, rows_per_block);
    PCRCG_CHECK_LAUNCH();
    return PCRCG_OK;
}

size_t colstats_ws_bytes(int c) { return carve_bytes((size_t)kStatChunks * 2 * (size_t)(c > 0 ? c : 1), sizeof(double)); }

int colstats_finalize(const double* partial, int nchunks, int c, double count, float eps, float* stats,
                      hipStream_t st) {
    hipLaunchKernelGGL(k_colstats_final, dim3((c + 3) / 4), dim3(256), 0, st, partial, nchunks, c, count, eps, stats);
    PCRCG_CHECK_LAUNCH();
    return PCRCG_OK;
}
int colstats_chunks() { return kStatChunks; }

int gather_max_multi(const GatherJob* jobs, int count, int c, hipStream_t st) {
    PCRCG_CHECK_ARG(jobs && count >= 1 && count <= 4 && c >= 1);
    GatherMulti mm;
    bool vec = c % 4 == 0;
    int nq_max = 0;
    for (int g = 0; g < 4; ++g) {
        const GatherJob& j = jobs[g < count ? g : 0];
        mm.x[g] = j.x; mm.idx[g] = reinterpret_cast<const long long*>(j.idx); mm.out[g] = j.out;
        mm.ns[g] = j.ns; mm.nq[g] = g < count ? j.nq : 0; mm.h[g] = j.h; mm.ld_idx[g] = j.ld_idx;
        mm.walk[g] = j.walk;
        if (g < count) {
            PCRCG_CHECK_ARG((j.walk != nullptr) == (jobs[0].walk != nullptr));
            PCRCG_CHECK_ARG(j.ns >= 0 && j.nq >= 0 && j.h >= 1 && j.ld_idx >= j.h && (j.nq == 0 || (j.x && j.idx && j.out)));
            vec = vec && ((reinterpret_cast<uintptr_t>(j.x) | reinterpret_cast<uintptr_t>(j.out)) & 15) == 0;
            nq_max = j.nq > nq_max ? j.nq : nq_max;
        }
    }
    if (nq_max == 0) return PCRCG_OK;
    const int per_wave = vec ? 256 : 64;
    const int nchunk = (c + per_wave - 1) / per_wave;
    const long items = jobs[0].walk ? (long)((nq_max + 7) / 8) * nchunk : (long)nq_max * nchunk;
    const dim3 grid((unsigned)((items + kWavesPerBlock - 1) / kWavesPerBlock) * (jobs[0].walk ? 8 : 1), count);
    if (vec) hipLaunchKernelGGL(k_gather_max<true>, grid, dim3(kWavesPerBlock * 64), 0, st, mm, c, nchunk);
    else hipLaunchKernelGGL(k_gather_max<false>, grid, dim3(kWavesPerBlock * 64), 0, st, mm, c, nchunk);
    PCRCG_CHECK_LAUNCH();
    return PCRCG_OK;
}

int gather_first_multi(const FirstJob* jobs, int count, int c, int ld_x, int ld_out, hipStream_t st) {
    PCRCG_CHECK_ARG(jobs && count >= 1 && count <= 4 && c >= 1 && ld_x >= c && ld_out >= c);
    FirstMulti mm;
    bool vec = ld_x % 4 == 0 && ld_out % 4 == 0;
    int nq_max = 0;
    for (int g = 0; g < 4; ++g) {
        const FirstJob& j = jobs[g < count ? g : 0];
        mm.x[g] = j.x; mm.idx[g] = reinterpret_cast<const long long*>(j.idx); mm.out[g] = j.out;
        mm.ns[g] = j.ns; mm.nq[g] = g < count ? j.nq : 0; mm.ld_idx[g] = j.ld_idx;
        if (g < count) {
            PCRCG_CHECK_ARG(j.ns >= 0 && j.nq >= 0 && j.ld_idx >= 1 && (j.nq == 0 || (j.idx && j.out && (j.x || j.ns == 0))));
            if (j.nq > 0) vec = vec && ((reinterpret_cast<uintptr_t>(j.x) | reinterpret_cast<uintptr_t>(j.out)) & 15) == 0;
            nq_max = j.nq > nq_max ? j.nq : nq_max;
        }
    }
    if (nq_max == 0) return PCRCG_OK;
    const long threads = (long)nq_max * ((c + 3) / 4);
    const dim3 grid((unsigned)((threads + 255) / 256), count);
    if (vec) hipLaunchKernelGGL(k_gather_first_multi<true>, grid, dim3(256), 0, st, mm, c, ld_x, ld_out);
    else hipLaunchKernelGGL(k_gather_first_multi<false>, grid, dim3(256), 0, st, mm, c, ld_x, ld_out);
    PCRCG_CHECK_LAUNCH();
    return PCRCG_OK;
}

int instnorm_colsums_multi(const float* const* x, double* const* sums, const int* n, int count, int c, int ldx, hipStream_t st) {
    PCRCG_CHECK_ARG(count >= 1 && count <= 4 && c >= 1 && ldx >= c);
    ColsMulti mm;
    int nmax = 0;
    for (int g = 0; g < 4; ++g) {
        const int k = g < count ? g : 0;
        PCRCG_CHECK_ARG(n[k] >= 1 && x[k] && sums[k]);
        mm.x[g] = x[k]; mm.partial[g] = sums[k]; mm.n[g] = n[k];
        if (g < count) nmax = n[k] > nmax ? n[k] : nmax;
    }
    int chunks = (nmax + 63) / 64;
    if (chunks > kStatChunks) chunks = kStatChunks;
    if (debug_opts().deterministic) chunks = 1;
    hipLaunchKernelGGL(k_colstats_partial<true>, dim3(chunks, (c + 63) / 64, count), dim3(256), 0, st, mm, c, ldx);
    PCRCG_CHECK_LAUNCH();
    return PCRCG_OK;
}

}

using namespace pcrcg;

extern "C" {

int pcrcg_gather_max(const float* x, int ns, int c, const int64_t* idx, int nq, int h, int ld_idx,
                     float* out, void* stream) {
    PCRCG_CHECK_ARG(ns >= 0 && c >= 1 && nq >= 0 && h >= 1 && ld_idx >= h);
    if (nq == 0) return PCRCG_OK;
    PCRCG_CHECK_ARG(x && idx && out);
    const GatherJob one{x, idx, out, ns, nq, h, ld_idx};
    return gather_max_multi(&one, 1, c, as_stream(stream));
}

int pcrcg_gather_first(const float* x, int ns, int c, const int64_t* idx, int nq, int ld_idx, float* out,
                       int ld_out, void* stream) {
    PCRCG_CHECK_ARG(ns >= 0 && c >= 1 && nq >= 0 && ld_idx >= 1 && ld_out >= c);
    if (nq == 0) return PCRCG_OK;
    PCRCG_CHECK_ARG(x && idx && out);
    hipLaunchKernelGGL(k_gather_first, dim3((nq + 3) / 4), dim3(256), 0, as_stream(stream), x, ns, c,
                       reinterpret_cast<const long long*>(idx), nq, ld_idx, out, ld_out);
    PCRCG_CHECK_LAUNCH();
    return PCRCG_OK;
}

int pcrcg_gather_first_multi(const float* const* x, const int* ns, const int64_t* const* idx, const int* nq, const int* ld_idx,
                             float* const* out, int count, int c, int ld_x, int ld_out, void* stream) {
    PCRCG_CHECK_ARG(x && ns && idx && nq && ld_idx && out && count >= 1 && count <= 4);
    FirstJob jobs[4];
    for (int g = 0; g < count; ++g) jobs[g] = FirstJob{x[g], idx[g], out[g], ns[g], nq[g], ld_idx[g]};
    return gather_first_multi(jobs, count, c, ld_x, ld_out, as_stream(stream));
}

size_t pcrcg_instnorm_ws_bytes(int c) { return colstats_ws_bytes(c); }

int pcrcg_instnorm_stats_from_partials(const void* partials, int chunks, int c, double count, float eps,
                                       float* stats, void* stream) {
    PCRCG_CHECK_ARG(partials && stats && chunks >= 1 && c >= 1 && count >= 1.0);
    return colstats_finalize(static_cast<const double*>(partials), chunks, c, count, eps, stats, as_stream(stream));
}

int pcrcg_instnorm_stats(const float* x, int n, int c, int ldx, float eps, float* stats, void* ws,
                         size_t ws_bytes, void* stream) {
    PCRCG_CHECK_ARG(n >= 1 && c >= 1 && ldx >= c && x && stats && ws);
    Carver cv(ws, ws_bytes);
    double* partial = cv.take<double>((size_t)kStatChunks * 2 * c);
    PCRCG_CHECK_WS(cv);
    hipStream_t st = as_stream(stream);
    {
        ColsMulti mm;
        for (int g = 0; g < 4; ++g) { mm.x[g] = x; mm.partial[g] = partial; mm.n[g] = n; }
        hipLaunchKernelGGL(k_colstats_partial<false>, dim3(kStatChunks, (c + 63) / 64, 1), dim3(256), 0, st, mm, c, ldx);
    }
    return colstats_finalize(partial, kStatChunks, c, (double)n, eps, stats, st);
}

int pcrcg_instnorm_colsums(const float* x, int n, int c, int ldx, void* sums, void* stream) {
    PCRCG_CHECK_ARG(n >= 1 && c >= 1 && ldx >= c && x && sums);
    const float* xs[1] = {x};
    double* ss[1] = {static_cast<double*>(sums)};
    return instnorm_colsums_multi(xs, ss, &n, 1, c, ldx, as_stream(stream));
}

int pcrcg_instnorm_apply_sums(const float* x, int n, int c, int ldx, const void* sums, double count, float eps,
                              const float* res, int ldr, const void* res_sums, float slope, float* y, int ldy,
                              void* stream) {
    PCRCG_CHECK_ARG(n >= 0 && c >= 4 && c % 4 == 0 && ldx >= c && ldy >= c && count >= 1.0);
    if (n == 0) return PCRCG_OK;
    PCRCG_CHECK_ARG(x && sums && y && (!res || ldr >= c) && (!res_sums || res));
    auto al16 = [](const void* p) { return (reinterpret_cast<uintptr_t>(p) & 15) == 0; };
    PCRCG_CHECK_ARG(instnorm_sums_ok(c, ldx, ldy, res ? ldr : 0) && al16(x) && al16(y) && (!res || al16(res)));
    NormJob one{x, static_cast<const double*>(sums), res, static_cast<const double*>(res_sums), y, nullptr, nullptr, n, count};
    return instnorm_apply_sums_multi(&one, 1, c, ldx, eps, ldr, slope, ldy, false, as_stream(stream));
}

int pcrcg_instnorm_apply(const float* x, int n, int c, int ldx, const float* stats, const float* res,
                         int ldr, const float* res_stats, float slope, float* y, int ldy, void* stream) {
    PCRCG_CHECK_ARG(n >= 0 && c >= 1 && ldx >= c && ldy >= c);
    if (n == 0) return PCRCG_OK;
    PCRCG_CHECK_ARG(x && stats && y);
    PCRCG_CHECK_ARG(!res || ldr >= c);
    auto al16 = [](const void* p) { return (reinterpret_cast<uintptr_t>(p) & 15) == 0; };
    const bool vec = c % 4 == 0 && ldx % 4 == 0 && ldy % 4 == 0 && al16(x) && al16(y) && al16(stats) &&
// ... 15 lines not shown
```

### pcrcg_amd/csrc/runner.hip

```cpp
#include <vector>

#include <cstdlib>

#include "gemm.h"

namespace pcrcg {
namespace {

constexpr int GMAX = 4;
static_assert(GMAX <= 4, "instnorm_apply_sums_multi, instnorm_colsums_multi, gather_max_multi, gather_first_multi, copy2d_multi, heads_multi, "
                         "edgeconv_rows_multi and attention_mfma_multi (common.h) take up to four clouds");

struct Mat {
    float* p[GMAX] = {};
    int rows[GMAX] = {};
    int cols = 0, ld = 0;
    bool zeroed = false;
};

struct Ctx {
    char* base = nullptr;
    size_t cap = 0, off = 0, peak = 0;
    hipStream_t st = nullptr;
    bool dry = false;
// ... 165 lines not shown
    }
    for (int g = 0; g < c.G; ++g) {
        const NormJob& j = jobs[g];
        c.check(pcrcg_instnorm_apply_sums(j.x, j.n, cols, ldx, j.sums, j.count, 1e-5f, j.res, ldr, j.res_sums, slope, j.y, ldy, c.st));
    }
}

void norm_act(Ctx& c, const Mat& x, float slope, const Mat& y, Stat* xs = nullptr, const Mat* res = nullptr,
              bool norm_res = false, Stat* rs = nullptr) {
    fill_sums(c, x, xs);
    if (res && norm_res) fill_sums(c, *res, rs);
    if (c.live() && all_sums(c, xs) && (!res || !norm_res || all_sums(c, rs)) && sums_apply_ok(x, y, res)) {
        const NormJobs nj = norm_jobs(c, x, xs->partials, y, res, (res && norm_res) ? rs->partials : nullptr);
        apply_sums(c, nj.j, nj.aligned, x.cols, x.ld, res ? res->ld : 0, slope, y.ld);
        return;
    }
    const size_t m = c.mark();
    float* stats = static_cast<float*>(c.raw(sizeof(float) * 2 * x.cols));
    float* rstats = (res && norm_res) ? static_cast<float*>(c.raw(sizeof(float) * 2 * x.cols)) : nullptr;
    const size_t wsb = pcrcg_instnorm_ws_bytes(x.cols);
    void* ws = c.raw(wsb);
    if (c.live())
        for (int g = 0; g < c.G; ++g) {
            col_stats(c, x, g, xs, stats, ws, wsb);
            if (rstats) col_stats(c, *res, g, rs, rstats, ws, wsb);
            c.check(pcrcg_instnorm_apply(x.p[g], x.rows[g], x.cols, x.ld, stats, res ? res->p[g] : nullptr, res ? res->ld : 0,
                                         rstats, slope, y.p[g], y.ld, c.st));
        }
    c.release(m);
}

void stats_into(GemmCall& call, Stat* st, int g) {
    if (!st) return;
    call.colstats = st->partials[g];
    call.colstats_bytes = st->bytes;
    call.h_chunks = &st->chunks[g];
    call.colstats_sums = st->sums;
}
struct Fold {
    Stat* sums = nullptr;
    float slope = 1.0f;
    bool accumulate = false;
};
GemmExtra extra_of(const Fold& f, const Mat& x, int g) {
    GemmExtra ex;
    if (f.sums) {
        ex.a_sums = static_cast<const double*>(f.sums->partials[g]);
        ex.a_count = (double)x.rows[g];
        ex.a_slope = f.slope;
    }
    ex.accumulate = f.accumulate;
    return ex;
}
GemmGroup group_of(const Ctx& c, const Mat& x, const Mat& y, bool c_zeroed, Stat* st, const float* const* row_scale, const Fold* f) {
    GemmGroup grp;
    grp.n = c.G - 1;
    for (int g = 1; g < c.G; ++g) {
        GemmPair& p = grp.p[g - 1];
        p.a = x.p[g];
        p.c = y.p[g];
        p.m = x.rows[g];
        p.row_scale = row_scale ? row_scale[g] : nullptr;
        p.colstats = st ? st->partials[g] : nullptr;
        p.h_chunks = st ? &st->chunks[g] : nullptr;
        p.c_zeroed = c_zeroed;
        if (f && f->sums) { p.a_sums = static_cast<const double*>(f->sums->partials[g]); p.a_count = (double)x.rows[g]; }
    }
    return grp;
}

void linear(Ctx& c, const Mat& x, const float* w, int ldw, const float* bias, const Mat& y, bool c_zeroed, Stat* st = nullptr,
            const float* const* row_scale = nullptr, const Fold* f = nullptr) {
    if (!c.live()) return;
    const bool grouped = c.paired();
    for (int g = 0; g < (grouped ? 1 : c.G); ++g) {
        GemmCall call;
        call.a = x.p[g]; call.lda = x.ld;
        call.b = w; call.ldb = ldw;
        call.c = y.p[g]; call.ldc = y.ld;
        call.m = x.rows[g]; call.n = y.cols; call.k = x.cols;
        call.row_scale = row_scale ? row_scale[g] : nullptr;
        call.bias = bias;
        call.st = c.st;
        stats_into(call, st, g);
        call.c_zeroed = c_zeroed;
        const GemmExtra ex = f ? extra_of(*f, x, g) : GemmExtra();
        const GemmGroup grp = grouped ? group_of(c, x, y, c_zeroed, st, row_scale, f) : GemmGroup();
        if (f) call.ex = &ex;
        if (grouped) call.grp = &grp;
        c.check(gemm_run(call));
    }
}
void linear(Ctx& c, const Mat& x, const float* w, int ldw, const float* bias, const Mat& y, Stat* st = nullptr,
            const float* const* row_scale = nullptr) {
    linear(c, x, w, ldw, bias, y, y.zeroed, st, row_scale);
}

bool lazy_stats_ready(Ctx& c, const Mat& x, Stat* xs) {
    if (!xs || !xs->sums || x.ld % 4 != 0 || x.cols > 4096) return false;
    fill_sums(c, x, xs);
    return true;
}
bool linear_norm(Ctx& c, const Mat& x, Stat* xs, float slope, const float* w, int ldw, const float* bias, const Mat& y,
                 Stat* st = nullptr) {
    if (!gemm_split_terms_on() || !lazy_stats_ready(c, x, xs)) return false;
    Fold f;
    f.sums = xs;
    f.slope = slope;
    linear(c, x, w, ldw, bias, y, y.zeroed, st, nullptr, &f);
    return true;
}

struct Batches { const pcrcg_batch* b[GMAX]; };

struct Walks {
    int* w[PCRCG_MAX_LEVELS][GMAX] = {};
    bool built[PCRCG_MAX_LEVELS] = {};
    int mode = 0;
};

static bool walk_pays(int mode, int ns, int cin, int nq) {
    if (mode != 1) return mode == 2;
    return (size_t)ns * (size_t)cin * sizeof(float) > (size_t)8 << 20 && nq >= 2048;
}

const int* const* level_walks(Ctx& c, const Batches& B, Walks& W, int l) {
    if (c.live() && !W.built[l]) {
        const float* pts[GMAX];
        int n[GMAX];
        for (int g = 0; g < c.G; ++g) { pts[g] = B.b[g]->points[l]; n[g] = B.b[g]->n_points[l]; }
        c.check(query_walk_multi(pts, n, W.w[l], nullptr, c.G, c.st));
        W.built[l] = true;
    }
    return W.w[l];
}

int kp_cin(const pcrcg_block& blk, const Mat& x) { return (blk.kp_w_pad && blk.cin_pad > x.cols) ? blk.cin_pad : x.cols; }
const float* kp_weight(const pcrcg_block& blk, const Mat& x) {
    return (blk.kp_w_pad && blk.cin_pad > 0 && kp_cin(blk, x) == blk.cin_pad) ? blk.kp_w_pad : blk.kp_w;
}

int kp_k(const pcrcg_block& blk, const Mat& x) {
    const int cin = kp_cin(blk, x);
    return (cin == 1 && blk.kp_wt) ? 16 : PCRCG_KPOINTS * cin;
}

void kpconv(Ctx& c, const Batches& B, Walks& W, const pcrcg_block& blk, const Mat& x, const Mat& y, Stat* st = nullptr,
            void* const* packed_ws = nullptr) {
    const int l = blk.layer;
    const size_t m = c.mark();
    Mat xin = x;
    const float* const w = kp_weight(blk, x);
    const int cin = kp_cin(blk, x);
    if (cin > x.cols) {
        xin = c.mat(x.rows, cin);
        if (c.live())
            for (int g = 0; g < c.G; ++g) {
                c.check(hipMemsetAsync(xin.p[g], 0, sizeof(float) * (size_t)x.rows[g] * cin, c.st) == hipSuccess ? PCRCG_OK
                                                                                                                   : PCRCG_ELAUNCH);
                c.check(pcrcg_copy2d(x.p[g], x.ld, xin.p[g], cin, x.rows[g], x.cols, c.st));
            }
    }
    int nq[GMAX], ns[GMAX];
    const float* q[GMAX];
    const pcrcg_table* tab[GMAX];
    float* inv_n[GMAX];
    void* ws[GMAX];
    size_t wsb[GMAX];
    for (int g = 0; g < c.G; ++g) {
        const pcrcg_batch& b = *B.b[g];
        tab[g] = blk.strided ? &b.pools[l] : &b.neighbors[l];
        q[g] = blk.strided ? b.points[l + 1] : b.points[l];
        nq[g] = blk.strided ? b.n_points[l + 1] : b.n_points[l];
        ns[g] = b.n_points[l];
        inv_n[g] = static_cast<float*>(c.raw(sizeof(float) * (nq[g] > 0 ? nq[g] : 1)));
        wsb[g] = pcrcg_kpconv_ws_bytes(ns[g]);
// ... 64 lines not shown
Mat simple_block(Ctx& c, const Batches& B, Walks& W, const pcrcg_block& blk, const Mat& x) {
    int nq[GMAX];
    out_rows(c, B, blk, nq);
    Mat y = c.mat(nq, blk.mid_dim);
    const size_t m = c.mark();
    Mat t = c.gemm_out(nq, y.cols, kp_k(blk, x));
    Stat ts = stat_buffer(c, nq, t.cols);
    kpconv(c, B, W, blk, x, t, &ts);
    norm_act(c, t, 0.1f, y, &ts);
    c.release(m);
    return y;
}

bool norm_act_pack(Ctx& c, const Batches& B, int layer, const Mat& t, float slope, const Mat& u, Stat* ts, void* const* kp_ws,
                   const size_t* kp_ws_bytes) {
    if (c.bf16 || !instnorm_pack_ok(t.cols, t.ld, u.ld) || u.ld != u.cols) return false;
    const size_t m = c.mark();
    float* stats = static_cast<float*>(c.raw(sizeof(float) * 2 * t.cols));
    const size_t wsb = pcrcg_instnorm_ws_bytes(t.cols);
    void* ws = c.raw(wsb);
    fill_sums(c, t, ts);
    if (c.live() && all_sums(c, ts)) {
        NormJobs nj = norm_jobs(c, t, ts->partials, u);
        bool ok = nj.aligned;
        for (int g = 0; g < c.G; ++g) {
            nj.j[g].s_pts = B.b[g]->points[layer];
            nj.j[g].pk = kpconv_pk_ptr(kp_ws[g], kp_ws_bytes[g], t.rows[g]);
            ok = ok && nj.j[g].pk != nullptr;
        }
        if (ok) {
            c.check(instnorm_apply_sums_multi(nj.j, c.G, t.cols, t.ld, 1e-5f, 0, slope, u.ld, true, c.st));
            c.release(m);
            return true;
        }
    }
    if (c.live())
        for (int g = 0; g < c.G; ++g) {
            const float* s_pts = B.b[g]->points[layer];
            float4* pk = kpconv_pk_ptr(kp_ws[g], kp_ws_bytes[g], t.rows[g]);
            if (!pk) c.check(PCRCG_EWORKSPACE);
            else if (ts && ts->has_sums(g))
                c.check(instnorm_apply_pack(t.p[g], t.rows[g], t.cols, t.ld, nullptr, static_cast<const double*>(ts->partials[g]),
                                            (double)t.rows[g], 1e-5f, slope, u.p[g], u.ld, s_pts, pk, c.st));
            else {
                col_stats(c, t, g, ts, stats, ws, wsb);
                c.check(instnorm_apply_pack(t.p[g], t.rows[g], t.cols, t.ld, stats, nullptr, 0.0, 1e-5f, slope, u.p[g], u.ld, s_pts,
                                            pk, c.st));
            }
        }
    c.release(m);
    return true;
}

Mat resnet_block(Ctx& c, const Batches& B, Walks& W, const pcrcg_block& blk, const Mat& feats) {
    int nq[GMAX];
    out_rows(c, B, blk, nq);
    Mat y = c.mat(nq, blk.out_dim);
    const size_t m = c.mark();
    Mat x = feats;
    void* kp_ws[GMAX] = {};
    size_t kp_wsb[GMAX] = {};
    bool packed = false;
    if (blk.unary1) {
        Mat t = c.gemm_out(feats.rows, blk.mid_dim, feats.cols), u = c.mat(feats.rows, blk.mid_dim);
        Stat ts = stat_buffer(c, t.rows, t.cols);
        linear(c, feats, blk.unary1, feats.cols, nullptr, t, &ts);
        if (blk.mid_dim % 4 == 0 && !(blk.kp_w_pad && blk.cin_pad > blk.mid_dim)) {
            for (int g = 0; g < c.G; ++g) {
                kp_wsb[g] = pcrcg_kpconv_ws_bytes(feats.rows[g]);
                kp_ws[g] = c.raw(kp_wsb[g]);
            }
            packed = norm_act_pack(c, B, blk.layer, t, 0.1f, u, &ts, kp_ws, kp_wsb);
        }
        if (!packed) norm_act(c, t, 0.1f, u, &ts);
        x = u;
    }
    Mat k = c.gemm_out(nq, blk.mid_dim, PCRCG_KPOINTS * kp_cin(blk, x)), kn = c.mat(nq, blk.mid_dim);
    Stat ks = stat_buffer(c, nq, blk.mid_dim);
    kpconv(c, B, W, blk, x, k, &ks, packed ? kp_ws : nullptr);
    Mat u2 = c.gemm_out(nq, blk.out_dim, blk.mid_dim);
    Stat u2s = stat_buffer(c, nq, blk.out_dim);
    if (!linear_norm(c, k, &ks, 0.1f, blk.unary2, blk.mid_dim, nullptr, u2, &u2s)) {
        norm_act(c, k, 0.1f, kn, &ks);
        linear(c, kn, blk.unary2, blk.mid_dim, nullptr, u2, &u2s);
    }
    Mat sc = feats;
    if (blk.strided) {
        sc = c.mat(nq, feats.cols);
        if (c.live()) {
            GatherJob jobs[GMAX];
            const int* const* walks = walk_pays(W.mode, c.max_rows(feats.rows), feats.cols, c.max_rows(nq)) ? level_walks(c, B, W, blk.layer + 1) : nullptr;
            for (int g = 0; g < c.G; ++g) {
                const pcrcg_table& t = B.b[g]->pools[blk.layer];
                jobs[g] = GatherJob{feats.p[g], t.idx, sc.p[g], feats.rows[g], nq[g], t.cols, t.ld, walks ? walks[g] : nullptr};
            }
            c.check(gather_max_multi(jobs, c.G, feats.cols, c.st));
        }
    }
    if (blk.shortcut) {
        Mat s2 = c.gemm_out(nq, blk.out_dim, sc.cols);
        Stat s2s = stat_buffer(c, nq, blk.out_dim);
        linear(c, sc, blk.shortcut, sc.cols, nullptr, s2, &s2s);
        norm_act(c, u2, 0.1f, y, &u2s, &s2, true, &s2s);
    } else {
        norm_act(c, u2, 0.1f, y, &u2s, &sc, false);
    }
    c.release(m);
    return y;
}

void edge_norm(Ctx& c, const float* cn, int ld_cn, int cw, const int* idx, int n, int k, float* emax, int ld_emax, float* out,
               int ld_out, void* sums, bool sums_ok, float* stats, void* ws, size_t wsb) {
    if (sums && sums_ok) {
        c.check(pcrcg_edgeconv_reduce_sums(cn, ld_cn, cn + cw, ld_cn, idx, n, k, cw, emax, ld_emax, sums, c.st));
        c.check(pcrcg_instnorm_apply_sums(emax, n, cw, ld_emax, sums, (double)n * (double)k, 1e-5f, nullptr, 0, nullptr, 0.2f, out,
                                          ld_out, c.st));
        return;
    }
    c.check(pcrcg_edgeconv_reduce(cn, ld_cn, cn + cw, ld_cn, idx, n, k, cw, 1e-5f, emax, ld_emax, stats, ws, wsb, c.st));
    c.check(pcrcg_instnorm_apply(emax, n, cw, ld_emax, stats, nullptr, 0, nullptr, 0.2f, out, ld_out, c.st));
}

void edge_norm_all(Ctx& c, const Mat& cn, int cw, int* const* idx, const int* n, const int* k, const Mat& e, const Mat& out,
                   void* const* sums, bool sums_ok, float* stats, void* ws, size_t wsb) {
    bool multi = sums_ok;
    EdgeCloud cl[GMAX];
    for (int g = 0; g < c.G; ++g) {
        multi = multi && sums[g] != nullptr;
        cl[g] = EdgeCloud{cn.p[g], cn.p[g] + cw, idx[g], e.p[g], static_cast<double*>(sums[g]), n[g], k[g]};
    }
    if (multi && edgeconv_rows_ok(cl, c.G, cn.ld, cn.ld, e.ld, cw)) {
        c.check(edgeconv_rows_multi(cl, c.G, cn.ld, cn.ld, e.ld, cw, true, nullptr, c.st));
        NormJobs nj = norm_jobs(c, e, sums, out);
        bool one = nj.aligned;
        for (int g = 0; g < c.G; ++g) {
            nj.j[g].count = (double)n[g] * (double)k[g];
            one = one && n[g] > 0 && k[g] > 0;
        }
        apply_sums(c, nj.j, one, cw, e.ld, 0, 0.2f, out.ld);
        return;
    }
    for (int g = 0; g < c.G; ++g)
        edge_norm(c, cn.p[g], cn.ld, cw, idx[g], n[g], k[g], e.p[g], e.ld, out.p[g], out.ld, sums[g], sums_ok, stats, ws, wsb);
}

Mat self_attention(Ctx& c, const pcrcg_model& mdl, const pcrcg_gnn_layer& gl, const float* const* coords, const Mat& f,
                   int* const* knn_given = nullptr) {
    const int ch = f.cols;
    Mat y = c.mat(f.rows, ch);
    const size_t m = c.mark();
    int kq[GMAX];
    int* idx[GMAX];
    for (int g = 0; g < c.G; ++g) {
        const int n = f.rows[g];
        kq[g] = mdl.knn_k < n - 1 ? mdl.knn_k : n - 1;
// ... 59 lines not shown
            c.check(attention_mfma_multi(cl, c.G, q.ld, kk.ld, v.ld, msg.ld, h, d, 1.0f / sqrtf((float)d), c.st));
            att_done = true;
        }
    }
    if (c.live())
        for (int g = 0; g < c.G; ++g) {
            const int n = x.rows[g], ms = src.rows[g];
            if (att_done) {
            } else if (pcrcg_attention_supported(d) && (long)n * ms <= 1000000) {
                c.check(pcrcg_attention(q.p[g], q.ld, kk.p[g], kk.ld, v.p[g], v.ld, msg.p[g], msg.ld, n, ms, h, d,
                                        1.0f / sqrtf((float)d), c.st));
            } else {
                for (int i = 0; i < h; ++i) {
                    c.check(pcrcg_gemm_f32(q.p[g] + i * d, q.ld, kk.p[g] + i * d, kk.ld, 1, sc.p[g], ms, n, ms, d, nullptr, nullptr,
                                           c.st));
                    c.check(pcrcg_softmax_rows(sc.p[g], n, ms, ms, 1.0f / sqrtf((float)d), c.st));
                    c.check(pcrcg_gemm_f32(sc.p[g], ms, v.p[g] + i * d, v.ld, 0, msg.p[g] + i * d, msg.ld, n, d, ms, nullptr, nullptr,
                                           c.st));
                }
            }
        }
    if (c.live()) c.check(copy2d_multi(x.p, cat.p, x.rows, c.G, x.ld, cat.ld, ch, c.st));
    linear(c, msg, gl.wm, ch, gl.bm, cols(cat, ch, ch));
    Stat h0s = stat_buffer(c, x.rows, 2 * ch);
    linear(c, cat, gl.w0, 2 * ch, gl.b0, h0, &h0s);
    if (!linear_norm(c, h0, &h0s, 0.0f, gl.w3, 2 * ch, gl.b3, delta)) {
        norm_act(c, h0, 0.0f, h1, &h0s);
        linear(c, h1, gl.w3, 2 * ch, gl.b3, delta);
    }
    if (c.live())
        for (int g = 0; g < c.G; ++g) c.check(pcrcg_add(x.p[g], delta.p[g], y.p[g], (long)x.rows[g] * ch, c.st));
    c.release(m);
    return y;
}

void forward(Ctx& c, const pcrcg_model& mdl, const Batches& B, const pcrcg_outputs* out) {
    const int L = B.b[0]->n_levels;
    c.bf16 = mdl.feature_bf16 != 0;
    Mat x;
    for (int g = 0; g < c.G; ++g) {
        x.p[g] = const_cast<float*>(B.b[g]->features);
        x.rows[g] = B.b[g]->n_points[0];
    }
    x.cols = x.ld = B.b[0]->feat_dim;
    std::vector<Mat> skips;
    Walks W;
    W.mode = debug_opts().walk;
    if (W.mode)
        for (int l = 0; l < L; ++l)
            for (int g = 0; g < c.G; ++g) {
                const int n = B.b[g]->n_points[l];
                W.w[l][g] = static_cast<int*>(c.raw(sizeof(int) * (size_t)(n > 0 ? n : 1)));
            }
    for (int i = 0; i < mdl.n_enc; ++i) {
        if (mdl.enc_skip[i]) skips.push_back(x);
        const pcrcg_block& blk = mdl.enc[i];
        x = blk.type == PCRCG_BLK_SIMPLE ? simple_block(c, B, W, blk, x) : resnet_block(c, B, W, blk, x);
    }
    const int gd = mdl.gnn_dim;
    int nc[GMAX] = {}, ns[GMAX] = {}, nt[GMAX] = {}, zero[GMAX] = {};
    const float *c0[GMAX], *c1[GMAX];
    for (int g = 0; g < c.G; ++g) {
        nc[g] = B.b[g]->n_points[L - 1];
        ns[g] = B.b[g]->len_src_c;
        nt[g] = nc[g] - ns[g];
        c0[g] = B.b[g]->points[L - 1];
        c1[g] = B.b[g]->points[L - 1] + 3 * (long)ns[g];
    }
    Mat fc = c.gemm_out(nc, gd, mdl.enc_out_dim);
    linear(c, x, mdl.bottle_w, mdl.enc_out_dim, mdl.bottle_b, fc);
    Mat d0 = rows(fc, zero, ns), d1 = rows(fc, ns, nt);
    int* knn0[GMAX] = {};
    int* knn1[GMAX] = {};
    int n_self = 0;
    for (int i = 0; i < mdl.n_gnn; ++i) n_self += mdl.gnn[i].cross ? 0 : 1;
    const bool knn_once = n_self >= 2;
    if (knn_once)
        for (int g = 0; g < c.G; ++g) {
            const int k0 = mdl.knn_k < ns[g] - 1 ? mdl.knn_k : ns[g] - 1, k1 = mdl.knn_k < nt[g] - 1 ? mdl.knn_k : nt[g] - 1;
            knn0[g] = static_cast<int*>(c.raw(sizeof(int) * (size_t)ns[g] * (k0 > 0 ? k0 : 1)));
            knn1[g] = static_cast<int*>(c.raw(sizeof(int) * (size_t)nt[g] * (k1 > 0 ? k1 : 1)));
            if (c.live()) {
                c.check(pcrcg_knn(c0[g], ns[g], k0, knn0[g], c.st));
                c.check(pcrcg_knn(c1[g], nt[g], k1, knn1[g], c.st));
            }
        }
    const int G0 = c.G;
    const bool stack = 2 * G0 <= GMAX && gemm_split_terms_on();
    const float* c01[GMAX] = {};
    int* knn01[GMAX] = {};
    for (int g = 0; g < G0 && stack; ++g) { c01[g] = c0[g]; c01[G0 + g] = c1[g]; knn01[g] = knn0[g]; knn01[G0 + g] = knn1[g]; }
    for (int i = 0; i < mdl.n_gnn; ++i) {
        const pcrcg_gnn_layer& gl = mdl.gnn[i];
        if (gl.cross) {
            Mat q0, q1;
            if (stack) {
                const int ch = d0.cols;
                const Mat x2 = stacked(d0, d1, G0);
                const Mat q2 = c.twice([&] { Mat q = c.gemm_out(x2.rows, ch, ch); linear(c, x2, gl.wq, ch, gl.bq, q); return q; });
                q0 = half(q2, 0, G0);
                q1 = half(q2, 1, G0);
            }
            d0 = cross_attention(c, mdl, gl, d0, d1, stack ? &q0 : nullptr);
            d1 = cross_attention(c, mdl, gl, d1, d0, stack ? &q1 : nullptr);
        } else if (stack) {
            const Mat f2 = stacked(d0, d1, G0);
            const Mat y2 = c.twice([&] { return self_attention(c, mdl, gl, c01, f2, knn_once ? knn01 : nullptr); });
            d0 = half(y2, 0, G0);
            d1 = half(y2, 1, G0);
        } else {
// ... 4 lines not shown
    const int wc = gd + 2;
    Mat xc = c.mat(nc, wc, pad4(wc));
    {
        const size_t m = c.mark();
        Mat gcat = c.mat(nc, gd), fn = c.mat(nc, gd);
        Mat pst = c.mat(ns, c.max_rows(nt)), pts = c.mat(nt, c.max_rows(ns));
        if (c.live())
            for (int g = 0; g < c.G; ++g) {
                c.check(pcrcg_copy2d(d0.p[g], d0.ld, gcat.p[g], gcat.ld, ns[g], gd, c.st));
                c.check(pcrcg_copy2d(d1.p[g], d1.ld, gcat.p[g] + (long)ns[g] * gcat.ld, gcat.ld, nt[g], gd, c.st));
            }
        Mat feats = cols(xc, 2, gd), score = cols(xc, 0, 1), sal = cols(xc, 1, 1);
        linear(c, gcat, mdl.proj_gnn_w, gd, mdl.proj_gnn_b, feats);
        linear(c, feats, mdl.proj_score_w, gd, mdl.proj_score_b, score);
        if (c.live())
            for (int g = 0; g < c.G; ++g) {
                c.check(pcrcg_l2norm_rows(feats.p[g], feats.ld, fn.p[g], fn.ld, nc[g], gd, c.st));
                const float inv_t = 1.0f / mdl.temperature;
                const float* fs = fn.p[g];
                const float* ft = fn.p[g] + (long)ns[g] * fn.ld;
                c.check(pcrcg_gemm_f32(fs, fn.ld, ft, fn.ld, 1, pst.p[g], nt[g], ns[g], nt[g], gd, nullptr, nullptr, c.st));
                c.check(pcrcg_softmax_matvec(pst.p[g], ns[g], nt[g], nt[g], inv_t, score.p[g] + (long)ns[g] * xc.ld, xc.ld, sal.p[g],
                                             xc.ld, c.st));
                c.check(pcrcg_gemm_f32(ft, fn.ld, fs, fn.ld, 1, pts.p[g], ns[g], nt[g], ns[g], gd, nullptr, nullptr, c.st));
                c.check(pcrcg_softmax_matvec(pts.p[g], nt[g], ns[g], ns[g], inv_t, score.p[g], xc.ld, sal.p[g] + (long)ns[g] * xc.ld,
                                             xc.ld, c.st));
            }
        c.release(m);
    }
    x = xc;
    Stat xs;
    bool lazy = false;
    auto materialise = [&]() {
        if (!lazy) return;
        Mat y = c.mat(x.rows, x.cols);
        norm_act(c, x, 0.1f, y, &xs);
        x = y;
        lazy = false;
    };
    for (int j = 0; j < mdl.n_dec; ++j) {
        const pcrcg_block& blk = mdl.dec[j];
        if (blk.type == PCRCG_BLK_UPSAMPLE) {
            const pcrcg_table* tabs[GMAX];
            int trows[GMAX] = {};
            for (int g = 0; g < c.G; ++g) { tabs[g] = &B.b[g]->upsamples[blk.layer - 1]; trows[g] = tabs[g]->rows; }
            const bool concat = j + 1 < mdl.n_dec && mdl.dec_concat[j + 1];
            const int cs = concat ? skips.back().cols : 0;
            const pcrcg_block* next = j + 1 < mdl.n_dec ? &mdl.dec[j + 1] : nullptr;
            if (concat && next && next->mlp_skip && next->skip_dim == cs && gemm_split_terms_on() &&
                (next->type == PCRCG_BLK_UNARY || next->type == PCRCG_BLK_LAST_UNARY) && x.ld % 4 == 0 &&
                skips.back().ld % 4 == 0) {
                const Mat& sk = skips.back();
                const bool last = next->type == PCRCG_BLK_LAST_UNARY;
                Mat tt = c.mat(trows, next->out_dim, pad4(next->out_dim));
                if (lazy && !(gemm_split_terms_on() && lazy_stats_ready(c, x, &xs))) materialise();
                Mat z = c.gemm_out(x.rows, next->out_dim, x.cols, pad4(next->out_dim));
                Fold up, add;
                up.sums = lazy ? &xs : nullptr;
                up.slope = 0.1f;
                add.accumulate = true;
                linear(c, x, next->mlp, next->mlp_ld, nullptr, z, z.zeroed, nullptr, nullptr, &up);
                if (c.live()) {
                    FirstJob jobs[GMAX];
                    for (int g = 0; g < c.G; ++g) jobs[g] = FirstJob{z.p[g], tabs[g]->idx, tt.p[g], z.rows[g], trows[g], tabs[g]->ld};
                    c.check(gather_first_multi(jobs, c.G, z.cols, z.ld, tt.ld, c.st));
                }
                linear(c, sk, next->mlp_skip, next->mlp_skip_ld, nullptr, tt, true, nullptr, nullptr, &add);
                skips.pop_back();
                lazy = false;
                x = tt;
                if (!last) {
                    xs = stat_buffer(c, tt.rows, tt.cols);
                    lazy = true;
                }
                ++j;
                continue;
            }
            materialise();
            Mat y = c.mat(trows, x.cols + cs, pad4(x.cols + cs));
            Mat xd = x;
            if (x.ld != x.cols) {
                xd = c.mat(x.rows, x.cols);
                if (c.live())
                    for (int g = 0; g < c.G; ++g) c.check(pcrcg_copy2d(x.p[g], x.ld, xd.p[g], xd.ld, x.rows[g], x.cols, c.st));
            }
            if (c.live())
                for (int g = 0; g < c.G; ++g) {
                    c.check(pcrcg_gather_first(xd.p[g], xd.rows[g], xd.cols, tabs[g]->idx, tabs[g]->rows, tabs[g]->ld, y.p[g], y.ld, c.st));
                    if (concat) {
                        const Mat& s = skips.back();
                        c.check(pcrcg_copy2d(s.p[g], s.ld, y.p[g] + x.cols, y.ld, s.rows[g], s.cols, c.st));
                    }
                }
            if (concat) skips.pop_back();
            x = y;
        } else if (blk.type == PCRCG_BLK_UNARY) {
            materialise();
            Mat t = c.gemm_out(x.rows, blk.out_dim, x.cols), y = c.mat(x.rows, blk.out_dim);
            Stat ts = stat_buffer(c, t.rows, t.cols);
            linear(c, x, blk.mlp, blk.mlp_ld, nullptr, t, &ts);
            norm_act(c, t, 0.1f, y, &ts);
            x = y;
        } else {
            materialise();
            Mat y = c.mat(x.rows, blk.out_dim, pad4(blk.out_dim));
            linear(c, x, blk.mlp, blk.mlp_ld, nullptr, y);
            x = y;
        }
    }
    materialise();
    if (c.live()) {
        const int fd = mdl.final_dim;
        float *ff[GMAX], *so[GMAX], *ss[GMAX];
        for (int g = 0; g < c.G; ++g) { ff[g] = out[g].feats_f; so[g] = out[g].scores_overlap; ss[g] = out[g].scores_saliency; }
        c.check(heads_multi(x.p, x.rows, c.G, x.ld, fd, ff, so, ss, c.st));
    }
}

int validate(const pcrcg_model* m, const pcrcg_batch* b) {
    PCRCG_CHECK_ARG(m && b);
    PCRCG_CHECK_ARG(m->n_enc >= 1 && m->n_enc <= PCRCG_MAX_BLOCKS && m->n_dec >= 1 && m->n_dec <= PCRCG_MAX_BLOCKS);
    PCRCG_CHECK_ARG(m->n_gnn >= 0 && m->n_gnn <= PCRCG_MAX_GNN);
    PCRCG_CHECK_ARG(b->n_levels >= 1 && b->n_levels <= PCRCG_MAX_LEVELS);
    PCRCG_CHECK_ARG(b->len_src_c >= 1 && b->len_src_c < b->n_points[b->n_levels - 1]);
    PCRCG_CHECK_ARG(m->heads >= 1 && m->gnn_dim % m->heads == 0 && m->temperature > 0.0f);
    for (int i = 0; i < m->n_enc; ++i) PCRCG_CHECK_ARG(m->enc[i].layer >= 0 && m->enc[i].layer + m->enc[i].strided < b->n_levels);
    const pcrcg_block& b0 = m->enc[0];
    if (b->feat_dim != b0.in_dim && !(b0.kp_w_pad && b0.cin_pad > 0 && b->feat_dim == b0.cin_pad)) {
        set_error("pcrcg_kpfcnn_forward: bad argument: batch feat_dim %d is neither the first block's in_dim %d nor its cin_pad %d "
                  "(with kp_w_pad)", b->feat_dim, b0.in_dim, b0.kp_w_pad ? b0.cin_pad : 0);
        return PCRCG_EBADARG;
    }
    return PCRCG_OK;
}

int validate_group(const pcrcg_model* m, const pcrcg_batch* b, int n) {
    PCRCG_CHECK_ARG(b && n >= 1 && n <= GMAX);
    for (int g = 0; g < n; ++g) {
        PCRCG_PROPAGATE(validate(m, b + g));
        PCRCG_CHECK_ARG(b[g].n_levels == b[0].n_levels && b[g].feat_dim == b[0].feat_dim);
    }
    return PCRCG_OK;
}

}
}

// ... 52 lines not shown
```

### pcrcg_amd/csrc/scan.hip

```cpp
#include <cstring>

#include <atomic>
#include <mutex>
#include <vector>

#include "common.h"

namespace pcrcg {

static thread_local char g_err[512] = "";

void set_error(const char* fmt, ...) {
    va_list ap;
    va_start(ap, fmt);
    vsnprintf(g_err, sizeof(g_err), fmt, ap);
    va_end(ap);
}

namespace {

constexpr int kScanThreads = 256;
constexpr int kScanItems = 8;
constexpr int kScanTile = kScanThreads * kScanItems;

// ... 130 lines not shown
                if (base + i < n) out[base + i] = v[t][i];
        }
        __syncthreads();
    }
    if (total && threadIdx.x == 0) *total = carry;
}

__global__ void zero_int(int* p) { *p = 0; }

}

size_t scan_ws_bytes(int n) {
    int nt = n > 0 ? (n + kScanTile - 1) / kScanTile : 1;
    return carve_bytes((size_t)nt, sizeof(int));
}

int exclusive_scan_i32(const int* in, int* out, int n, int* total, void* ws, hipStream_t stream) {
    if (n <= 0) {
        if (total) hipLaunchKernelGGL(zero_int, dim3(1), dim3(1), 0, stream, total);
        PCRCG_CHECK_LAUNCH();
        return PCRCG_OK;
    }
    const int nt = (n + kScanTile - 1) / kScanTile;
    if (nt == 1) {
        hipLaunchKernelGGL(scan_apply, dim3(1), dim3(kScanThreads), 0, stream, in, out, n,
                           (const int*)nullptr, total);
        PCRCG_CHECK_LAUNCH();
        return PCRCG_OK;
    }
    if (n <= kOneTiles * kOneThreads * kScanItems && (reinterpret_cast<uintptr_t>(in) & 15) == 0 &&
        (reinterpret_cast<uintptr_t>(out) & 15) == 0) {
        hipLaunchKernelGGL(scan_one_block, dim3(1), dim3(kOneThreads), 0, stream, in, out, n, total);
        PCRCG_CHECK_LAUNCH();
        return PCRCG_OK;
    }
    int* partial = static_cast<int*>(ws);
    hipLaunchKernelGGL(scan_tile_sums, dim3(nt), dim3(kScanThreads), 0, stream, in, n, partial);
    hipLaunchKernelGGL(scan_partials, dim3(1), dim3(kScanThreads), 0, stream, partial, nt, total);
    hipLaunchKernelGGL(scan_apply, dim3(nt), dim3(kScanThreads), 0, stream, in, out, n,
                       (const int*)partial, (int*)nullptr);
    PCRCG_CHECK_LAUNCH();
    return PCRCG_OK;
}

namespace {
struct DebugName { const char* name; int DebugOpts::*field; };
const DebugName kDebugNames[] = {
    {"stat_sums", &DebugOpts::stat_sums}, {"stat_sums_rows", &DebugOpts::stat_sums_rows}, {"att_mfma", &DebugOpts::att_mfma},
    {"radius_blocks", &DebugOpts::radius_blocks}, {"kd_blocks", &DebugOpts::kd_blocks}, {"att_tq", &DebugOpts::att_tq},
    {"kd_spin_limit", &DebugOpts::kd_spin_limit}, {"gemm_log", &DebugOpts::gemm_log}, {"x6_tile", &DebugOpts::x6_tile}, {"x6_order", &DebugOpts::x6_order}, {"x6_big", &DebugOpts::x6_big}, {"x6_h2", &DebugOpts::x6_h2}, {"train_side_stream", &DebugOpts::train_side_stream},
    {"x6_splitk", &DebugOpts::x6_splitk}, {"x6_t1", &DebugOpts::x6_t1}, {"x6_t2", &DebugOpts::x6_t2},
    {"gemm_tile", &DebugOpts::gemm_tile}, {"gemm_splitk", &DebugOpts::gemm_splitk},
    {"gemm_split_target", &DebugOpts::gemm_split_target}, {"deterministic", &DebugOpts::deterministic},
    {"bwd_mfma", &DebugOpts::bwd_mfma}, {"walk", &DebugOpts::walk}};
std::atomic<const DebugOpts*> g_debug{nullptr};
std::atomic<const DebugOpts*> g_debug_env{nullptr};
std::once_flag g_debug_once;
std::mutex g_debug_set_lock;
const DebugOpts kDebugDefaults{};

bool debug_parse(const char* spec, const DebugOpts* base) {
    DebugOpts d = *base;
    const char* p = spec;
    while (p && *p) {
        const char* end = strchr(p, ',');
        const size_t len = end ? (size_t)(end - p) : strlen(p);
        const char* eq = static_cast<const char*>(memchr(p, '=', len));
        bool ok = false;
        if (eq) {
            for (const DebugName& n : kDebugNames)
                if (strlen(n.name) == (size_t)(eq - p) && strncmp(n.name, p, (size_t)(eq - p)) == 0) {
                    d.*(n.field) = atoi(eq + 1);
                    ok = true;
                }
        }
        if (!ok && len > 0) {
            set_error("pcrcg_debug_set: unknown or malformed item '%.*s'", (int)len, p);
            return false;
        }
        p = end ? end + 1 : nullptr;
    }
    if (d.deterministic) {
        d.stat_sums = 0;
        d.gemm_splitk = 1;
    }
    g_debug.store(new DebugOpts(d), std::memory_order_release);
    return true;
}
}

const DebugOpts& debug_opts() {
    std::call_once(g_debug_once, [] {
        g_debug.store(&kDebugDefaults, std::memory_order_release);
        if (const char* e = getenv("PCRCG_DEBUG"))
            if (!debug_parse(e, &kDebugDefaults)) fprintf(stderr, "libpcrcg_hip: PCRCG_DEBUG ignored: %s\n", g_err);
        g_debug_env.store(g_debug.load(std::memory_order_acquire), std::memory_order_release);
    });
    return *g_debug.load(std::memory_order_acquire);
}

static std::mutex g_scratch_lock;
static std::vector<StreamScratch*>& scratch_registry() {
    static std::vector<StreamScratch*> all;
    return all;
}
StreamScratch::StreamScratch(bool cleared) : cleared_(cleared) {
    std::lock_guard<std::mutex> g(g_scratch_lock);
// ... 65 lines not shown
```

### pcrcg_amd/ops.py

```python
import ctypes

import torch

from . import _lib

_F32, _I32, _I64 = torch.float32, torch.int32, torch.int64


def _stream():
    return torch.cuda.current_stream().cuda_stream


def _dev(t, dtype, name):
    if not isinstance(t, torch.Tensor) or not t.is_cuda:
        raise RuntimeError(f"pcrcg_amd: `{name}` must be a tensor on a HIP device (no CPU fallback exists)")
    if t.dtype != dtype:
        raise RuntimeError(f"pcrcg_amd: `{name}` must have dtype {dtype}, got {t.dtype}")
    return t


def _rows(t, dtype, name):
    _dev(t, dtype, name)
    if t.dim() != 2:
        raise RuntimeError(f"pcrcg_amd: `{name}` must be 2-D")
# ... 291 lines not shown
    b, ldb, trans_b = _operand_b(b)
    m, k = a.shape
    k2, n = b.shape
    if k != k2:
        raise RuntimeError(f"pcrcg_amd.gemm: inner dimensions differ ({k} vs {k2})")
    if out is None:
        out = torch.empty((m, n), dtype=_F32, device=a.device)
    out_, ldc = _rows(out, _F32, "out")
    if out_.data_ptr() != out.data_ptr():
        raise RuntimeError("pcrcg_amd.gemm: `out` must have unit inner stride")
    if row_scale is not None:
        row_scale = _dev(row_scale, _F32, "row_scale").contiguous()
    if bias is not None:
        bias = _dev(bias, _F32, "bias").contiguous()
    if grad_operand:
        _lib.check(L.pcrcg_gemm_f32_grad(a.data_ptr(), lda, int(trans_a), b.data_ptr(), ldb, trans_b, out.data_ptr(), ldc, m, n, k,
                                         _ptr(row_scale), _ptr(bias), int(grad_operand), _stream()), "pcrcg_gemm_f32_grad")
        return out
    if trans_a:
        _lib.check(L.pcrcg_gemm_f32_ex(a.data_ptr(), lda, 1, b.data_ptr(), ldb, trans_b, out.data_ptr(), ldc, m, n, k,
                                       _ptr(row_scale), _ptr(bias), _stream()), "pcrcg_gemm_f32_ex")
        return out
    _lib.check(L.pcrcg_gemm_f32(a.data_ptr(), lda, b.data_ptr(), ldb, trans_b, out.data_ptr(), ldc, m, n, k,
                                _ptr(row_scale), _ptr(bias), _stream()), "pcrcg_gemm_f32")
    return out


def gemm_fused(a, w, idx=None, out=None, accumulate=False, sums=None, slope=1.0, bias=None, eps=1e-5):
    L = _lib.lib()
    a, lda = _rows(a, _F32, "a")
    w, ldb = _rows(w, _F32, "w")
    k, n = a.shape[1], w.shape[0]
    if idx is not None:
        idx, ld_idx = _rows(idx, _I64, "idx")
        m = idx.shape[0]
    else:
        ld_idx, m = 0, a.shape[0]
    if out is None:
        if accumulate:
            raise RuntimeError("pcrcg_amd.gemm_fused: accumulate needs `out`")
        out = torch.empty((m, n), dtype=_F32, device=a.device)
    if sums is not None and (sums.dtype != torch.float64 or tuple(sums.shape) != (2, k) or not sums.is_contiguous()):
        raise RuntimeError("pcrcg_amd.gemm_fused: sums must be a contiguous float64 [2, k] tensor")
    if bias is not None:
        bias = _dev(bias, _F32, "bias").contiguous()
    zero = torch.zeros(k + 8, dtype=_F32, device=a.device)
    _lib.check(L.pcrcg_gemm_f32_fused(a.data_ptr(), lda, _ptr(idx), ld_idx, a.shape[0], zero.data_ptr(), _ptr(sums),
                                      float(a.shape[0]), float(eps), float(slope), w.data_ptr(), ldb, _ptr(bias),
                                      out.data_ptr(), out.stride(0) if m > 1 else max(n, out.stride(0)), m, n, k,
                                      int(accumulate), _stream()), "pcrcg_gemm_f32_fused")
    return out


def kpconv(q_pts, s_pts, idx, x, kernel_points, weights, extent):
    L = _lib.lib()
    q_pts = _dev(q_pts, _F32, "q_pts").contiguous()
    s_pts = _dev(s_pts, _F32, "s_pts").contiguous()
    idx, ld_idx = _rows(idx, _I64, "neighb_inds")
    x = _dev(x, _F32, "x").contiguous()
    kp = _dev(kernel_points, _F32, "kernel_points").contiguous()
    nq, h = idx.shape
    ns, cin = x.shape
    kdim = kp.shape[0]
    if kdim != 15:
        raise RuntimeError("pcrcg_amd.kpconv: only 15 kernel points are supported")
    if cin % 4 != 0 and cin > 4:
        pad = (-cin) % 4
        x = torch.nn.functional.pad(x, (0, pad))
        weights = torch.nn.functional.pad(weights, (0, 0, 0, pad))
        cin += pad
    wf = torch.empty((nq, kdim * cin), dtype=_F32, device=x.device)
    inv_n = torch.empty(nq, dtype=_F32, device=x.device)
    nbytes = L.pcrcg_kpconv_ws_bytes(ns)
    ws = _ws.get("kpconv", nbytes, x.device)
    w2 = _dev(weights, _F32, "weights").reshape(kdim * cin, -1)
    _lib.check(L.pcrcg_kpconv_aggregate(q_pts.data_ptr(), nq, s_pts.data_ptr(), ns, idx.data_ptr(), h, ld_idx,
                                        x.data_ptr(), cin, kp.data_ptr(), float(extent), wf.data_ptr(),
                                        inv_n.data_ptr(), ws.data_ptr(), nbytes, _stream()),
               "pcrcg_kpconv_aggregate")
    return gemm(wf, w2, row_scale=inv_n)


def kpconv_c1_layer(q_pts, s_pts, idx, x, kernel_points, wt, extent, out=None):
    L = _lib.lib()
    q_pts = _dev(q_pts, _F32, "q_pts").contiguous()
    s_pts = _dev(s_pts, _F32, "s_pts").contiguous()
    idx, ld_idx = _rows(idx, _I64, "neighb_inds")
    x = _dev(x, _F32, "x").contiguous()
    kp = _dev(kernel_points, _F32, "kernel_points").contiguous()
    wt = _dev(wt, _F32, "wt").contiguous()
    nq, h = idx.shape
    ns, cout = x.shape[0], wt.shape[0]
    if kp.shape[0] != 15 or wt.shape[1] != 16 or x.numel() != ns:
        raise RuntimeError("pcrcg_amd.kpconv_c1_layer: 15 kernel points, wt [cout, 16] and one feature per point")
    if out is None:
        out = torch.empty((nq, cout), dtype=_F32, device=x.device)
    ld_out = out.stride(0) if nq > 1 else max(cout, out.stride(0))
    inv_n = torch.empty(nq, dtype=_F32, device=x.device)
    sums = torch.zeros((2, cout), dtype=torch.float64, device=x.device)
    nbytes = L.pcrcg_kpconv_ws_bytes(ns)
    ws = _ws.get("kpconv", nbytes, x.device)
    _lib.check(L.pcrcg_kpconv_c1_layer(q_pts.data_ptr(), nq, s_pts.data_ptr(), ns, idx.data_ptr(), h, ld_idx, x.data_ptr(),
                                       kp.data_ptr(), float(extent), wt.data_ptr(), cout, out.data_ptr(), ld_out,
                                       inv_n.data_ptr(), sums.data_ptr(), ws.data_ptr(), nbytes, _stream()),
               "pcrcg_kpconv_c1_layer")
    return out, inv_n, sums
# ... 229 lines not shown
    return out


def gather_first(x, idx, out=None):
    L = _lib.lib()
    x = _dev(x, _F32, "x").contiguous()
    idx, ld_idx = _rows(idx, _I64, "inds")
    ns, c = x.shape
    nq = idx.shape[0]
    if out is None:
        out = torch.empty((nq, c), dtype=_F32, device=x.device)
    ld_out = out.stride(0) if nq > 1 else max(c, out.stride(0))
    if out.stride(1) != 1 and c > 1:
        raise RuntimeError("pcrcg_amd.gather_first: `out` must have unit inner stride")
    _lib.check(L.pcrcg_gather_first(x.data_ptr(), ns, c, idx.data_ptr(), nq, ld_idx, out.data_ptr(), ld_out,
                                    _stream()), "pcrcg_gather_first")
    return out


class NeighborTranspose:
    __slots__ = ("tq", "th", "deg", "n_edges", "d_max", "nq", "ns")

    def __init__(self, tq, th, deg, n_edges, d_max, nq, ns):
        self.tq, self.th, self.deg, self.n_edges, self.d_max, self.nq, self.ns = tq, th, deg, n_edges, d_max, nq, ns


def transpose_neighbors(idx, ns, with_columns=False, max_cols=None):
    L = _lib.lib()
    idx, ld_idx = _rows(idx, _I64, "inds")
    nq, h = idx.shape
    ns = int(ns)
    if h < 1:
        raise RuntimeError("pcrcg_amd.transpose_neighbors: the table needs at least one column")
    dev = idx.device
    deg = torch.empty(max(ns, 1), dtype=_I32, device=dev)[:ns]
    stats = torch.empty(2, dtype=_I32, device=dev)
    _lib.check(L.pcrcg_neighbors_transpose_count(idx.data_ptr(), nq, h, ld_idx, ns, deg.data_ptr(), stats.data_ptr(), _stream()),
               "pcrcg_neighbors_transpose_count")
    n_edges, d_max = (int(v) for v in stats.cpu())
    if max_cols is not None and d_max > max_cols:
        raise RuntimeError(f"pcrcg_amd.transpose_neighbors: d_max = {d_max} exceeds max_cols = {max_cols}")
    cols = max(d_max, 1)
    tq = torch.empty((ns, cols), dtype=_I64, device=dev)
    th = torch.empty((ns, cols), dtype=_I32, device=dev) if with_columns else None
    status = torch.empty(1, dtype=_I32, device=dev)
    nbytes = L.pcrcg_neighbors_transpose_ws_bytes(nq, h, ns)
    ws = _ws.get("transpose", nbytes, dev)
    _lib.check(L.pcrcg_neighbors_transpose_fill(idx.data_ptr(), nq, h, ld_idx, ns, deg.data_ptr(), cols, tq.data_ptr(), cols,
                                                _ptr(th), cols, status.data_ptr(), ws.data_ptr(), nbytes, _stream()),
               "pcrcg_neighbors_transpose_fill")
    return NeighborTranspose(tq, th, deg, n_edges, d_max, nq, ns)


def gather_first_multi(xs, idxs, outs):
    L = _lib.lib()
    n = len(xs)
    if not (1 <= n <= 4 and len(idxs) == n and len(outs) == n):
        raise RuntimeError("pcrcg_amd.gather_first_multi: one to four clouds")
    c = xs[0].shape[1]
    xs, ld_x = zip(*[_rows(x, _F32, "x") for x in xs])
    idxs, ld_idx = zip(*[_rows(i, _I64, "inds") for i in idxs])
    for o in outs:
        _dev(o, _F32, "out")
        if o.dim() != 2 or (o.shape[1] > 1 and o.stride(1) != 1):
            raise RuntimeError("pcrcg_amd.gather_first_multi: `out` must be 2-D with unit inner stride")
    ld_out = [o.stride(0) if o.shape[0] > 1 else max(c, o.stride(0)) for o in outs]
    many_x = [l for x, l in zip(xs, ld_x) if x.shape[0] > 1] or [max(ld_x)]
    many_o = [l for o, l in zip(outs, ld_out) if o.shape[0] > 1] or [max(ld_out)]
    if len(set(many_x)) != 1 or len(set(many_o)) != 1 or any(x.shape[1] != c for x in xs):
        raise RuntimeError("pcrcg_amd.gather_first_multi: the clouds must share width and leading dimensions")
    ptrs = lambda ts: (ctypes.c_void_p * n)(*[t.data_ptr() for t in ts])
    ints = lambda vs: (ctypes.c_int * n)(*[int(v) for v in vs])
    _lib.check(L.pcrcg_gather_first_multi(ptrs(xs), ints([x.shape[0] for x in xs]), ptrs(idxs), ints([i.shape[0] for i in idxs]),
                                          ints(ld_idx), ptrs(outs), n, c, many_x[0], many_o[0], _stream()),
               "pcrcg_gather_first_multi")
    return outs


def instnorm_stats(x, eps=1e-5):
    L = _lib.lib()
    x, ldx = _rows(x, _F32, "x")
    n, c = x.shape
    stats = torch.empty(2 * c, dtype=_F32, device=x.device)
    nbytes = L.pcrcg_instnorm_ws_bytes(c)
    ws = _ws.get("instnorm", nbytes, x.device)
    _lib.check(L.pcrcg_instnorm_stats(x.data_ptr(), n, c, ldx, float(eps), stats.data_ptr(), ws.data_ptr(), nbytes,
                                      _stream()), "pcrcg_instnorm_stats")
    return stats


def instnorm_apply(x, stats, slope=1.0, res=None, res_stats=None, out=None):
    L = _lib.lib()
    x, ldx = _rows(x, _F32, "x")
    n, c = x.shape
    ldr = 0
    if res is not None:
        res, ldr = _rows(res, _F32, "res")
    if out is None:
        out = torch.empty((n, c), dtype=_F32, device=x.device)
    ldy = out.stride(0) if n > 1 else max(c, out.stride(0))
    _lib.check(L.pcrcg_instnorm_apply(x.data_ptr(), n, c, ldx, stats.data_ptr(), _ptr(res), ldr, _ptr(res_stats),
                                      float(slope), out.data_ptr(), ldy, _stream()), "pcrcg_instnorm_apply")
    return out


def instnorm_colsums(x):
    L = _lib.lib()
    x, ldx = _rows(x, _F32, "x")
    sums = torch.zeros((2, x.shape[1]), dtype=torch.float64, device=x.device)
    if x.shape[0] > 0:
        _lib.check(L.pcrcg_instnorm_colsums(x.data_ptr(), x.shape[0], x.shape[1], ldx, sums.data_ptr(), _stream()),
                   "pcrcg_instnorm_colsums")
    return sums


def instnorm_apply_sums(x, sums, slope=1.0, res=None, res_sums=None, eps=1e-5, out=None, count=None):
    L = _lib.lib()
    x, ldx = _rows(x, _F32, "x")
    n, c = x.shape
    if sums.dtype != torch.float64 or tuple(sums.shape) != (2, c) or not sums.is_contiguous():
        raise RuntimeError("pcrcg_amd.instnorm_apply_sums: sums must be a contiguous float64 [2, c] tensor")
    ldr = 0
    if res is not None:
        res, ldr = _rows(res, _F32, "res")
    if out is None:
# ... 159 lines not shown
```

Measured before the change: 621.3.

## Fuse sibling GEMMs sharing an A operand and hoist decoder skip projection

Adds a sibling-GEMM path where two weight matrices that share the same A input run in one x6 kernel launch, with tiles past the first output width redirected to the second B/C/bias/colstats. In the encoder, the decoder's skip-projection GEMM is hoisted into the resnet block that already reads that skip input, and its result is later added during the gather-first upsampling via a new addend field. The aim is to cut kernel launches and repeated reads of A. The cost is more template variants and constraints: 64x64 tiles, no split-K, and the first width must be a multiple of the tile.

```diff
diff --git a/include/pcrcg.h b/include/pcrcg.h
--- a/include/pcrcg.h
+++ b/include/pcrcg.h
@@ -123,6 +123,11 @@
 int pcrcg_gemm_f32_fused(const float* a, int lda, const int64_t* idx, int ld_idx, int ns, const float* zero_row,
                          const void* a_sums, double a_count, float a_eps, float a_slope, const float* b, int ldb,
                          const float* bias, float* c, int ldc, int m, int n, int k, int accumulate, void* stream);
+int pcrcg_gemm_f32_sibling(int count, const float* const* a, const int* m, int lda, int k, const float* const* row_scale,
+                           const void* const* a_sums, float a_eps, float a_slope, const float* b0, int ldb0, int n0,
+                           const float* bias0, float* const* c0, int ldc0, void* const* stats0, const float* b1, int ldb1,
+                           int n1, const float* bias1, float* const* c1, int ldc1, void* const* stats1, int stats_sums,
+                           size_t stats_bytes, int* h_chunks, void* stream);
 
 void pcrcg_gemm_set_mode(int mode);
 int pcrcg_gemm_get_mode(void);
@@ -135,6 +140,9 @@
                        int ld_out, void* stream);
 int pcrcg_gather_first_multi(const float* const* x, const int* ns, const int64_t* const* idx, const int* nq, const int* ld_idx,
                              float* const* out, int count, int c, int ld_x, int ld_out, void* stream);
+int pcrcg_gather_first_add_multi(const float* const* x, const int* ns, const int64_t* const* idx, const int* nq, const int* ld_idx,
+                                 const float* const* addend, float* const* out, int count, int c, int ld_x, int ld_out,
+                                 void* stream);
 size_t pcrcg_instnorm_ws_bytes(int c);
 int pcrcg_instnorm_stats_from_partials(const void* partials, int chunks, int c, double count, float eps,
                                        float* stats, void* stream);
diff --git a/pcrcg_amd/_lib.py b/pcrcg_amd/_lib.py
--- a/pcrcg_amd/_lib.py
+++ b/pcrcg_amd/_lib.py
@@ -76,6 +76,10 @@
                                               c_void_p, c_void_p, c_void_p, c_size_t, c_void_p, c_void_p]),
     "pcrcg_gemm_f32_fused": (c_int, [c_void_p, c_int, c_void_p, c_int, c_int, c_void_p, c_void_p, ctypes.c_double, c_float,
                                      c_float, c_void_p, c_int, c_void_p, c_void_p, c_int, c_int, c_int, c_int, c_int, c_void_p]),
+    "pcrcg_gemm_f32_sibling": (c_int, [c_int, c_void_p, c_void_p, c_int, c_int, c_void_p, c_void_p, c_float, c_float,
+                                       c_void_p, c_int, c_int, c_void_p, c_void_p, c_int, c_void_p,
+                                       c_void_p, c_int, c_int, c_void_p, c_void_p, c_int, c_void_p,
+                                       c_int, c_size_t, c_void_p, c_void_p]),
     "pcrcg_gemm_set_mode": (None, [c_int]),
     "pcrcg_gemm_get_mode": (c_int, []),
     "pcrcg_gemm_redo_counts": (c_int, [c_void_p, c_int]),
@@ -83,6 +87,8 @@
                                                    c_void_p]),
     "pcrcg_gather_max": (c_int, [c_void_p, c_int, c_int, c_void_p, c_int, c_int, c_int, c_void_p, c_void_p]),
     "pcrcg_gather_first": (c_int, [c_void_p, c_int, c_int, c_void_p, c_int, c_int, c_void_p, c_int, c_void_p]),
+    "pcrcg_gather_first_add_multi": (c_int, [c_void_p, c_void_p, c_void_p, c_void_p, c_void_p, c_void_p, c_void_p, c_int, c_int, c_int,
+                                             c_int, c_void_p]),
     "pcrcg_gather_first_multi": (c_int, [c_void_p, c_void_p, c_void_p, c_void_p, c_void_p, c_void_p, c_int, c_int, c_int, c_int,
                                          c_void_p]),
     "pcrcg_instnorm_ws_bytes": (c_size_t, [c_int]),
diff --git a/pcrcg_amd/csrc/common.h b/pcrcg_amd/csrc/common.h
--- a/pcrcg_amd/csrc/common.h
+++ b/pcrcg_amd/csrc/common.h
@@ -86,7 +86,7 @@
 
 struct GatherJob { const float* x; const int64_t* idx; float* out; int ns, nq, h, ld_idx; const int* walk = nullptr; };
 int gather_max_multi(const GatherJob* jobs, int count, int c, hipStream_t st);
-struct FirstJob { const float* x; const int64_t* idx; float* out; int ns, nq, ld_idx; };
+struct FirstJob { const float* x; const int64_t* idx; float* out; int ns, nq, ld_idx; const float* addend = nullptr; };
 int gather_first_multi(const FirstJob* jobs, int count, int c, int ld_x, int ld_out, hipStream_t st);
 int heads_multi(const float* const* x, const int* rows, int count, int ld, int fd, float* const* feats, float* const* s_ov,
                 float* const* s_sal, hipStream_t st);
@@ -125,6 +125,7 @@
     int deterministic = 0;
     int bwd_mfma = 1;
     int walk = 1;
+    int siblings = 3;
 };
 const DebugOpts& debug_opts();
 
diff --git a/pcrcg_amd/csrc/gemm.h b/pcrcg_amd/csrc/gemm.h
--- a/pcrcg_amd/csrc/gemm.h
+++ b/pcrcg_amd/csrc/gemm.h
@@ -26,10 +26,25 @@
     int a_ns = 0;
     const double* a_sums = nullptr;
     double a_count = 0.0;
+    float* sib_c = nullptr;
+    void* sib_colstats = nullptr;
+    int* sib_h_chunks = nullptr;
 };
 struct GemmGroup {
     int n = 0;
     GemmPair p[3];
+};
+
+struct GemmSibling {
+    const float* b = nullptr;
+    int ldb = 0;
+    float* c = nullptr;
+    int ldc = 0, n = 0;
+    const float* bias = nullptr;
+    void* colstats = nullptr;
+    size_t colstats_bytes = 0;
+    int* h_chunks = nullptr;
+    bool c_zeroed = false;
 };
 
 enum class GemmA { row_f32, kmajor_f32, row_bf16 };
@@ -52,6 +67,7 @@
     bool c_zeroed = false;
     const GemmExtra* ex = nullptr;
     const GemmGroup* grp = nullptr;
+    const GemmSibling* sib = nullptr;
     hipStream_t st = nullptr;
 };
 
@@ -61,6 +77,7 @@
 
 int gemm_x6_dispatch(const GemmCall& g);
 int gemm_x6_splits(int m, int n, int k, long m_total);
+bool gemm_x6_sibling_ok(int m, int n, int n_sib, int k, long m_total, bool a_norm);
 int gemm_x6_redo_counts(unsigned long long* out, int reset);
 bool gemm_x6_shared();
 void gemm_x6_set_shared(int on);
diff --git a/pcrcg_amd/csrc/gemm.hip b/pcrcg_amd/csrc/gemm.hip
--- a/pcrcg_amd/csrc/gemm.hip
+++ b/pcrcg_amd/csrc/gemm.hip
@@ -378,12 +378,15 @@
     if (g.h_chunks) *g.h_chunks = 0;
     const bool trans_a = g.a_form == GemmA::kmajor_f32, b_kn = g.b_form == GemmB::kn, bf16 = g.a_form == GemmA::row_bf16;
     const bool grouped = g.grp && g.grp->n != 0;
-    const bool x6_form = g.ex || grouped || bf16;
+    const GemmSibling* const sib = (g.sib && g.sib->n > 0) ? g.sib : nullptr;
+    if (g.sib && g.sib->h_chunks) *g.sib->h_chunks = 0;
+    const bool x6_form = g.ex || grouped || bf16 || sib;
     PCRCG_CHECK_ARG(g.m >= 0 && g.n >= 0 && g.k >= 0);
     const bool ld_ok = (trans_a ? g.lda >= g.m : g.lda >= g.k) && (b_kn ? g.ldb >= g.n : g.ldb >= g.k) && g.ldc >= g.n;
     if (x6_form) PCRCG_CHECK_ARG(g.k >= 1 && ld_ok && !(trans_a && !b_kn));
     if (grouped) PCRCG_CHECK_ARG(g.m >= 1 && g.n >= 1);
     if (bf16) PCRCG_CHECK_ARG(g.k % 32 == 0 && g.lda % 8 == 0);
+    if (sib) PCRCG_CHECK_ARG(!bf16 && !trans_a && !b_kn && g.m >= 1 && g.n >= 1 && sib->b && sib->c && sib->ldb >= g.k && sib->ldc >= sib->n);
     if (g.m == 0 || g.n == 0) return PCRCG_OK;
     PCRCG_CHECK_ARG(g.a && g.b && g.c);
     PCRCG_CHECK_ARG(ld_ok);
@@ -468,6 +471,62 @@
     return gemm_run(g);
 }
 
+extern "C" int pcrcg_gemm_f32_sibling(int count, const float* const* a, const int* m, int lda, int k, const float* const* row_scale,
+                                      const void* const* a_sums, float a_eps, float a_slope, const float* b0, int ldb0, int n0,
+                                      const float* bias0, float* const* c0, int ldc0, void* const* stats0, const float* b1, int ldb1,
+                                      int n1, const float* bias1, float* const* c1, int ldc1, void* const* stats1, int stats_sums,
+                                      size_t stats_bytes, int* h_chunks, void* stream) {
+    PCRCG_CHECK_ARG(count >= 1 && count <= 4 && a && m && c0 && b0 && n0 >= 1 && n1 >= 0 && k >= 1);
+    PCRCG_CHECK_ARG(n1 == 0 || (b1 && c1));
+    PCRCG_CHECK_ARG(!(stats0 || stats1) || h_chunks);
+    if (!gemm_split_terms_on()) {
+        set_error("pcrcg_gemm_f32_sibling: only the split-bf16 arithmetic (pcrcg_gemm_set_mode(1)) implements it");
+        return PCRCG_EBADARG;
+    }
+    for (int g = 0; g < count; ++g) {
+        PCRCG_CHECK_ARG(m[g] >= 0);
+        if (h_chunks) h_chunks[g] = h_chunks[count + g] = 0;
+    }
+    int idx[4], cnt = 0;
+    for (int g = 0; g < count; ++g)
+        if (m[g] > 0) idx[cnt++] = g;
+    if (cnt == 0) return PCRCG_OK;
+    const int f = idx[0];
+    GemmCall g = plain_call(a[f], lda, 0, b0, ldb0, 1, c0[f], ldc0, m[f], n0, k, row_scale ? row_scale[f] : nullptr, bias0, stream);
+    if (stats0) { g.colstats = stats0[f]; g.colstats_bytes = stats_bytes; g.h_chunks = &h_chunks[f]; }
+    g.colstats_sums = stats_sums != 0;
+    GemmExtra ex;
+    if (a_sums) {
+        ex.a_sums = static_cast<const double*>(a_sums[f]);
+        ex.a_count = (double)m[f];
+        ex.a_eps = a_eps;
+        ex.a_slope = a_slope;
+        g.ex = &ex;
+    }
+    GemmSibling sib;
+    if (n1 > 0) {
+        sib.b = b1; sib.ldb = ldb1; sib.c = c1[f]; sib.ldc = ldc1; sib.n = n1; sib.bias = bias1;
+        if (stats1) { sib.colstats = stats1[f]; sib.colstats_bytes = stats_bytes; sib.h_chunks = &h_chunks[count + f]; }
+        g.sib = &sib;
+    }
+    GemmGroup grp;
+    grp.n = cnt - 1;
+    for (int i = 1; i < cnt; ++i) {
+        const int e = idx[i];
+        GemmPair& p = grp.p[i - 1];
+        p.a = a[e]; p.c = c0[e]; p.m = m[e];
+        p.row_scale = row_scale ? row_scale[e] : nullptr;
+        if (stats0) { p.colstats = stats0[e]; p.h_chunks = &h_chunks[e]; }
+        if (a_sums) { p.a_sums = static_cast<const double*>(a_sums[e]); p.a_count = (double)m[e]; }
+        if (n1 > 0) {
+            p.sib_c = c1[e];
+            if (stats1) { p.sib_colstats = stats1[e]; p.sib_h_chunks = &h_chunks[count + e]; }
+        }
+    }
+    if (grp.n > 0) g.grp = &grp;
+    return gemm_run(g);
+}
+
 extern "C" int pcrcg_gemm_f32_ex(const float* a, int lda, int trans_a, const float* b, int ldb, int trans_b, float* c,
                                  int ldc, int m, int n, int k, const float* row_scale, const float* bias, void* stream) {
     return gemm_run(plain_call(a, lda, trans_a, b, ldb, trans_b, c, ldc, m, n, k, row_scale, bias, stream));
diff --git a/pcrcg_amd/csrc/gemm_x6.hip b/pcrcg_amd/csrc/gemm_x6.hip
--- a/pcrcg_amd/csrc/gemm_x6.hip
+++ b/pcrcg_amd/csrc/gemm_x6.hip
@@ -36,6 +36,15 @@
     const double* a_sums[kGroupExtra] = {nullptr, nullptr, nullptr};
     double a_count[kGroupExtra] = {0.0, 0.0, 0.0};
 };
+struct GemmSibArgs {
+    const float* b = nullptr;
+    const float* bias = nullptr;
+    int ldb = 0, n = 0, ldc = 0;
+    float* c[1 + kGroupExtra] = {nullptr, nullptr, nullptr, nullptr};
+    double* colp[1 + kGroupExtra] = {nullptr, nullptr, nullptr, nullptr};
+    int colp_chunks[1 + kGroupExtra] = {0, 0, 0, 0};
+};
+struct NoSib {};
 
 __device__ __forceinline__ void gload16(f32x4& dst, const float* p) {
     asm volatile("global_load_dwordx4 %0, %1, off" : "=v"(dst) : "v"(p) : "memory");
@@ -130,7 +139,7 @@
     return cost1 < 0.9 * cost0 ? 1 : 0;
 }
 
-template <int BM, int BN, int MINB, int ATERMS, int ALAY, int BLAY, int ANORM = 0, int KNOCK = 0, int H2 = 0>
+template <int BM, int BN, int MINB, int ATERMS, int ALAY, int BLAY, int ANORM = 0, int KNOCK = 0, int H2 = 0, class SB = NoSib>
 __global__ void __launch_bounds__((x6_threads<BM, BN>()), MINB) k_gemm_x6(const float* __restrict__ A, int lda, const float* __restrict__ B,
                                                         int ldb, float* __restrict__ C, int ldc, int M, int N, int Kdim,
                                                         const float* __restrict__ row_scale,
@@ -139,7 +148,8 @@
                                                         int colp_chunks, const long long* __restrict__ a_idx,
                                                         int a_idx_ld, int a_ns, const float* __restrict__ a_zero,
                                                         const double* __restrict__ a_sums, double a_count, float a_eps,
-                                                        float a_slope, GemmPairArgs pr, TileMap tm, float h2_sa, float h2_sb) {
+                                                        float a_slope, GemmPairArgs pr, TileMap tm, float h2_sa, float h2_sb, SB sb) {
+    constexpr bool SIB = std::is_same<SB, GemmSibArgs>::value;
     constexpr int NT = x6_threads<BM, BN>();
     constexpr int WAVES_M = 2, WAVES_N = NT / 128;
     constexpr int WM = BM / WAVES_M, WN = BN / WAVES_N;
@@ -173,7 +183,8 @@
         tile_x = in_split / tm.gy;
     }
     int m0 = tile_y * BM;
-    const int n0 = tile_x * BN;
+    int n0 = tile_x * BN;
+    int prod = 0;
     if (pr.extra > 0 && m0 >= pr.off[0]) {
         int e = 0;
         if (pr.extra > 1 && m0 >= pr.off[1]) e = 1;
@@ -190,6 +201,20 @@
         a_ns = pr.a_ns[e];
         a_sums = pr.a_sums[e];
         a_count = pr.a_count[e];
+        prod = e + 1;
+    }
+    if constexpr (SIB) {
+        if (n0 >= N) {
+            n0 -= N;
+            B = sb.b;
+            ldb = sb.ldb;
+            N = sb.n;
+            C = sb.c[prod];
+            ldc = sb.ldc;
+            bias = sb.bias;
+            colp = sb.colp[prod];
+            colp_chunks = sb.colp_chunks[prod];
+        }
     }
     const int k_begin = split * k_per_split;
     const int k_end = min(Kdim, k_begin + k_per_split);
@@ -754,6 +779,7 @@
     GemmPairArgs pr;
     long split_stride = 0;
     float h2_sa = 1.f, h2_sb = 1.f;
+    GemmSibArgs sb;
 };
 
 template <int BM, int BN, int MINB, int ATERMS, int ALAY, int BLAY, int ANORM = 0, int KNOCK = 0, int H2 = 0>
@@ -773,7 +799,27 @@
     hipExtLaunchKernelGGL(kern, dim3(tm.gx * tm.gy * tm.gs), dim3(x6_threads<BM, BN>()), lds, st, prof.a, prof.b, 0, p.a, p.lda, p.b,
                           p.ldb, p.c, p.ldc, p.m, p.n, p.k, p.row_scale, p.bias, p.k_per_split, p.vec_a, p.vec_b, p.atomic_out,
                           p.colp, p.colp_chunks, p.a_idx, p.a_idx_ld, p.a_ns, p.a_zero, p.a_sums, p.a_count, p.a_eps, p.a_slope,
-                          p.pr, tm, p.h2_sa, p.h2_sb);
+                          p.pr, tm, p.h2_sa, p.h2_sb, NoSib());
+    PCRCG_CHECK_LAUNCH();
+    return PCRCG_OK;
+}
+template <int ANORM, int H2>
+int launch_x6_sib(const X6Args& p, dim3 grid, hipStream_t st) {
+    TileMap tm;
+    tm.split_stride = 0;
+    tm.gx = (int)grid.x;
+    tm.gy = (int)grid.y;
+    tm.gs = 1;
+    tm.order = x6_tile_order(tm.gx, tm.gy, 1, 64, 64, p.k_per_split);
+    const size_t lds = lds_bytes<64, 64>() + (ANORM ? 2 * sizeof(float) * (size_t)(((p.k_per_split + BK - 1) / BK) * BK) : 0) + (H2 ? 16 : 0);
+    auto kern = k_gemm_x6<64, 64, 4, 3, 0, 0, ANORM, 0, H2, GemmSibArgs>;
+    PCRCG_GRANT_LDS(kern);
+    int m_all = p.m;
+    for (int e = 0; e < p.pr.extra; ++e) m_all += p.pr.m[e];
+    KpProfScope prof(st, m_all, p.n + p.sb.n, p.k, H2 ? 3 : 6, 3);
+    hipExtLaunchKernelGGL(kern, dim3(tm.gx * tm.gy), dim3(256), lds, st, prof.a, prof.b, 0, p.a, p.lda, p.b, p.ldb, p.c, p.ldc, p.m, p.n, p.k,
+                          p.row_scale, p.bias, p.k_per_split, p.vec_a, p.vec_b, p.atomic_out, p.colp, p.colp_chunks, p.a_idx, p.a_idx_ld,
+                          p.a_ns, p.a_zero, p.a_sums, p.a_count, p.a_eps, p.a_slope, p.pr, tm, p.h2_sa, p.h2_sb, p.sb);
     PCRCG_CHECK_LAUNCH();
     return PCRCG_OK;
 }
@@ -836,6 +882,12 @@
 
 int gemm_x6_splits(int m, int n, int k, long m_total) { return (m > 0 && n > 0) ? x6_plan(m, n, k, false, false, m_total).splits : 1; }
 
+bool gemm_x6_sibling_ok(int m, int n, int n_sib, int k, long m_total, bool a_norm) {
+    if (m <= 0 || n <= 0 || n_sib <= 0 || k <= 0) return false;
+    const X6Plan plan = x6_plan(m, n + n_sib, k, a_norm, false, m_total);
+    return plan.pick == 3 && n % plan.bn == 0 && plan.splits == 1;
+}
+
 static int x6_run(const GemmCall& g, long split_stride) {
     const float* const a = static_cast<const float*>(g.a);
     const int m = g.m, n = g.n, k = g.k, ldc = g.ldc;
@@ -859,8 +911,25 @@
     const int grad_op = ex ? ex->grad_operand : 0;
     const bool h2 = debug_opts().x6_h2 != 0 && !a_bf16;
     const bool lifted = h2 && grad_op;
-    const X6Plan plan = x6_plan(m_plan, n, k, a_kmajor || b_kmajor || anorm || lifted, a_kmajor, m_total);
+    const GemmSibling* const sib = (g.sib && g.sib->n > 0) ? g.sib : nullptr;
+    const int n_sib = sib ? sib->n : 0;
+    const X6Plan plan = x6_plan(m_plan, n + n_sib, k, a_kmajor || b_kmajor || anorm || lifted, a_kmajor, m_total);
     const int BM = plan.bm, gx = plan.gx, splits = plan.splits;
+    if (sib) {
+        if (a_bf16 || a_kmajor || b_kmajor || accumulate || lifted || split_stride) {
+            set_error("gemm_x6: a sibling is built for k-contiguous fp32 operands without the accumulate and gradient forms");
+            return PCRCG_EBADARG;
+        }
+        if (plan.pick != 3 || n % plan.bn != 0) {
+            set_error("gemm_x6: a sibling needs the 64 x 64 tile and a first width that is a multiple of it (n = %d, tile %d x %d)", n,
+                      plan.bm, plan.bn);
+            return PCRCG_EBADARG;
+        }
+        if (splits > 1) {
+            set_error("gemm_x6: a sibling needs a plan without split-K (m = %d, n = %d + %d, k = %d: %d splits)", m, n, n_sib, k, splits);
+            return PCRCG_EBADARG;
+        }
+    }
     const int gy0 = (m + BM - 1) / BM;
     int gy = gy0, gye[kGroupExtra] = {0, 0, 0};
     for (int e = 0; e < n_extra; ++e) { gye[e] = (grp->p[e].m + BM - 1) / BM; gy += gye[e]; }
@@ -931,8 +1000,9 @@
     }
     const dim3 grid(gx, gy, splits);
     if (debug_opts().gemm_log != 0)
-        fprintf(stderr, "pcrcg_gemm_x6 m=%d n=%d k=%d lda=%d ldb=%d ldc=%d tile=%dx%d grid=%dx%dx%d rs=%d bias=%d stats=%d\n", m,
-                n, k, g.lda, g.ldb, ldc, BM, plan.bn, gx, gy, splits, g.row_scale != nullptr, g.bias != nullptr, g.colstats != nullptr);
+        fprintf(stderr, "pcrcg_gemm_x6 m=%d n=%d k=%d lda=%d ldb=%d ldc=%d tile=%dx%d grid=%dx%dx%d rs=%d bias=%d stats=%d sib=%d\n", m,
+                n, k, g.lda, g.ldb, ldc, BM, plan.bn, gx, gy, splits, g.row_scale != nullptr, g.bias != nullptr, g.colstats != nullptr,
+                n_sib);
     if (g.colstats && g.h_chunks && !p.atomic_out && g.colstats_sums) {
         if (2 * (size_t)n * sizeof(double) <= g.colstats_bytes) {
             p.colp = static_cast<double*>(g.colstats);
@@ -972,6 +1042,24 @@
             }
         }
     }
+    if (sib) {
+        GemmSibArgs& sb = p.sb;
+        sb.b = sib->b; sb.ldb = sib->ldb; sb.n = n_sib; sb.ldc = sib->ldc; sb.bias = sib->bias;
+        p.vec_b = p.vec_b && (sib->ldb % 4 == 0) && ((reinterpret_cast<uintptr_t>(sib->b) & 15) == 0);
+        for (int e = -1; e < n_extra; ++e) {
+            sb.c[e + 1] = e < 0 ? sib->c : grp->p[e].sib_c;
+            void* const cs = e < 0 ? sib->colstats : grp->p[e].sib_colstats;
+            int* const hc = e < 0 ? sib->h_chunks : grp->p[e].sib_h_chunks;
+            if (!sb.c[e + 1]) { set_error("gemm_x6: a product of the group has no sibling output"); return PCRCG_EBADARG; }
+            if (hc) *hc = 0;
+            if (!cs || !hc) continue;
+            const int chunks = g.colstats_sums ? -1 : (e < 0 ? gy0 : gye[e]) * 2;
+            const size_t need = g.colstats_sums ? 2 * (size_t)n_sib * sizeof(double) : carve_bytes(2 * (size_t)n_sib * chunks, sizeof(double));
+            if (need > sib->colstats_bytes) continue;
+            sb.colp[e + 1] = static_cast<double*>(cs);
+            sb.colp_chunks[e + 1] = *hc = chunks;
+        }
+    }
     if (gather) { p.a_idx = ex->a_idx; p.a_idx_ld = ex->a_idx_ld; p.a_ns = ex->a_ns; p.a_zero = ex->a_zero; }
     if (anorm) { p.a_sums = ex->a_sums; p.a_count = ex->a_count; p.a_eps = ex->a_eps; p.a_slope = ex->a_slope; }
     if (lifted && !anorm) { p.h2_sa = grad_op == 1 ? 65536.0f : 1.0f; p.h2_sb = grad_op == 2 ? 65536.0f : 1.0f; }
@@ -981,6 +1069,10 @@
         return lifted ? launch_x6<64, 64, 4, 3, 0, 1, 0, 0, 2>(p, grid, st) : launch_x6<64, 64, 4, 3, 0, 1>(p, grid, st);
     if (lifted && !anorm)
         return launch_x6<64, 64, 4, 3, 0, 0, 0, 0, 2>(p, grid, st);
+    if (sib) {
+        if (anorm) return h2 ? launch_x6_sib<1, 1>(p, grid, st) : launch_x6_sib<1, 0>(p, grid, st);
+        return h2 ? launch_x6_sib<0, 1>(p, grid, st) : launch_x6_sib<0, 0>(p, grid, st);
+    }
     if (anorm) return h2 ? launch_x6<64, 64, 4, 3, 0, 0, 1, 0, 1>(p, grid, st) : launch_x6<64, 64, 4, 3, 0, 0, 1>(p, grid, st);
     if (plan.pick == 0) return launch_x6_abt<128, 128, 2>(h2, a_bf16, p, grid, st);
     if (plan.pick == 1) return launch_x6_abt<128, 64, 2>(h2, a_bf16, p, grid, st);
diff --git a/pcrcg_amd/csrc/pointops.hip b/pcrcg_amd/csrc/pointops.hip
--- a/pcrcg_amd/csrc/pointops.hip
+++ b/pcrcg_amd/csrc/pointops.hip
@@ -74,8 +74,8 @@
     for (int cc = lane; cc < c; cc += 64) out[(long)q * ld_out + cc] = real ? x[i * c + cc] : 0.f;
 }
 
-struct FirstMulti { const float* x[4]; const long long* idx[4]; float* out[4]; int ns[4], nq[4], ld_idx[4]; };
-template <bool VEC>
+struct FirstMulti { const float* x[4]; const long long* idx[4]; float* out[4]; int ns[4], nq[4], ld_idx[4]; const float* addend[4]; };
+template <bool VEC, bool ADD>
 __global__ void __launch_bounds__(256) k_gather_first_multi(FirstMulti mm, int c, int ld_x, int ld_out) {
     const int g = blockIdx.y;
     const int segs = (c + 3) >> 2;
@@ -86,6 +86,19 @@
     const long long i = mm.idx[g][q * mm.ld_idx[g]];
     const bool real = i >= 0 && i < mm.ns[g];
     const float* __restrict__ src = mm.x[g] + (real ? i : 0) * ld_x + c0;
+    if constexpr (ADD) {
+        float* dst = mm.out[g] + q * ld_out + c0;
+        const float* add = mm.addend[g] + q * ld_out + c0;
+        if (VEC && c0 + 4 <= c) {
+            const float4 v = real ? *reinterpret_cast<const float4*>(src) : make_float4(0.f, 0.f, 0.f, 0.f);
+            const float4 a = *reinterpret_cast<const float4*>(add);
+            *reinterpret_cast<float4*>(dst) = make_float4(v.x + a.x, v.y + a.y, v.z + a.z, v.w + a.w);
+        } else {
+            const int n = c - c0 < 4 ? c - c0 : 4;
+            for (int k = 0; k < n; ++k) dst[k] = (real ? src[k] : 0.f) + add[k];
+        }
+        return;
+    }
     float* __restrict__ dst = mm.out[g] + q * ld_out + c0;
     if (VEC && c0 + 4 <= c) {
         *reinterpret_cast<float4*>(dst) = real ? *reinterpret_cast<const float4*>(src) : make_float4(0.f, 0.f, 0.f, 0.f);
@@ -441,22 +454,28 @@
     PCRCG_CHECK_ARG(jobs && count >= 1 && count <= 4 && c >= 1 && ld_x >= c && ld_out >= c);
     FirstMulti mm;
     bool vec = ld_x % 4 == 0 && ld_out % 4 == 0;
+    bool add = false;
+    for (int g = 0; g < count; ++g) add = add || (jobs[g].nq > 0 && jobs[g].addend);
     int nq_max = 0;
     for (int g = 0; g < 4; ++g) {
         const FirstJob& j = jobs[g < count ? g : 0];
         mm.x[g] = j.x; mm.idx[g] = reinterpret_cast<const long long*>(j.idx); mm.out[g] = j.out;
         mm.ns[g] = j.ns; mm.nq[g] = g < count ? j.nq : 0; mm.ld_idx[g] = j.ld_idx;
+        mm.addend[g] = j.addend;
         if (g < count) {
             PCRCG_CHECK_ARG(j.ns >= 0 && j.nq >= 0 && j.ld_idx >= 1 && (j.nq == 0 || (j.idx && j.out && (j.x || j.ns == 0))));
-            if (j.nq > 0) vec = vec && ((reinterpret_cast<uintptr_t>(j.x) | reinterpret_cast<uintptr_t>(j.out)) & 15) == 0;
+            PCRCG_CHECK_ARG((j.addend != nullptr) == add || j.nq == 0);
+            if (j.nq > 0) vec = vec && ((reinterpret_cast<uintptr_t>(j.x) | reinterpret_cast<uintptr_t>(j.out) | reinterpret_cast<uintptr_t>(j.addend)) & 15) == 0;
             nq_max = j.nq > nq_max ? j.nq : nq_max;
         }
     }
     if (nq_max == 0) return PCRCG_OK;
     const long threads = (long)nq_max * ((c + 3) / 4);
     const dim3 grid((unsigned)((threads + 255) / 256), count);
-    if (vec) hipLaunchKernelGGL(k_gather_first_multi<true>, grid, dim3(256), 0, st, mm, c, ld_x, ld_out);
-    else hipLaunchKernelGGL(k_gather_first_multi<false>, grid, dim3(256), 0, st, mm, c, ld_x, ld_out);
+    if (add && vec) hipLaunchKernelGGL((k_gather_first_multi<true, true>), grid, dim3(256), 0, st, mm, c, ld_x, ld_out);
+    else if (add) hipLaunchKernelGGL((k_gather_first_multi<false, true>), grid, dim3(256), 0, st, mm, c, ld_x, ld_out);
+    else if (vec) hipLaunchKernelGGL((k_gather_first_multi<true, false>), grid, dim3(256), 0, st, mm, c, ld_x, ld_out);
+    else hipLaunchKernelGGL((k_gather_first_multi<false, false>), grid, dim3(256), 0, st, mm, c, ld_x, ld_out);
     PCRCG_CHECK_LAUNCH();
     return PCRCG_OK;
 }
@@ -510,6 +529,17 @@
     PCRCG_CHECK_ARG(x && ns && idx && nq && ld_idx && out && count >= 1 && count <= 4);
     FirstJob jobs[4];
     for (int g = 0; g < count; ++g) jobs[g] = FirstJob{x[g], idx[g], out[g], ns[g], nq[g], ld_idx[g]};
+    return gather_first_multi(jobs, count, c, ld_x, ld_out, as_stream(stream));
+}
+
+int pcrcg_gather_first_add_multi(const float* const* x, const int* ns, const int64_t* const* idx, const int* nq, const int* ld_idx,
+                                 const float* const* addend, float* const* out, int count, int c, int ld_x, int ld_out, void* stream) {
+    PCRCG_CHECK_ARG(x && ns && idx && nq && ld_idx && addend && out && count >= 1 && count <= 4);
+    FirstJob jobs[4];
+    for (int g = 0; g < count; ++g) {
+        PCRCG_CHECK_ARG(addend[g] || nq[g] == 0);
+        jobs[g] = FirstJob{x[g], idx[g], out[g], ns[g], nq[g], ld_idx[g], addend[g]};
+    }
     return gather_first_multi(jobs, count, c, ld_x, ld_out, as_stream(stream));
 }
 
diff --git a/pcrcg_amd/csrc/runner.hip b/pcrcg_amd/csrc/runner.hip
--- a/pcrcg_amd/csrc/runner.hip
+++ b/pcrcg_amd/csrc/runner.hip
@@ -241,7 +241,15 @@
     ex.accumulate = f.accumulate;
     return ex;
 }
-GemmGroup group_of(const Ctx& c, const Mat& x, const Mat& y, bool c_zeroed, Stat* st, const float* const* row_scale, const Fold* f) {
+struct Sib {
+    const float* w = nullptr;
+    int ldw = 0;
+    const float* bias = nullptr;
+    Mat y;
+    Stat* st = nullptr;
+};
+GemmGroup group_of(const Ctx& c, const Mat& x, const Mat& y, bool c_zeroed, Stat* st, const float* const* row_scale, const Fold* f,
+                   const Sib* sb = nullptr) {
     GemmGroup grp;
     grp.n = c.G - 1;
     for (int g = 1; g < c.G; ++g) {
@@ -254,12 +262,17 @@
         p.h_chunks = st ? &st->chunks[g] : nullptr;
         p.c_zeroed = c_zeroed;
         if (f && f->sums) { p.a_sums = static_cast<const double*>(f->sums->partials[g]); p.a_count = (double)x.rows[g]; }
+        if (sb) {
+            p.sib_c = sb->y.p[g];
+            p.sib_colstats = sb->st ? sb->st->partials[g] : nullptr;
+            p.sib_h_chunks = sb->st ? &sb->st->chunks[g] : nullptr;
+        }
     }
     return grp;
 }
 
 void linear(Ctx& c, const Mat& x, const float* w, int ldw, const float* bias, const Mat& y, bool c_zeroed, Stat* st = nullptr,
-            const float* const* row_scale = nullptr, const Fold* f = nullptr) {
+            const float* const* row_scale = nullptr, const Fold* f = nullptr, const Sib* sb = nullptr) {
     if (!c.live()) return;
     const bool grouped = c.paired();
     for (int g = 0; g < (grouped ? 1 : c.G); ++g) {
@@ -274,9 +287,19 @@
         stats_into(call, st, g);
         call.c_zeroed = c_zeroed;
         const GemmExtra ex = f ? extra_of(*f, x, g) : GemmExtra();
-        const GemmGroup grp = grouped ? group_of(c, x, y, c_zeroed, st, row_scale, f) : GemmGroup();
+        const GemmGroup grp = grouped ? group_of(c, x, y, c_zeroed, st, row_scale, f, sb) : GemmGroup();
         if (f) call.ex = &ex;
         if (grouped) call.grp = &grp;
+        GemmSibling sib;
+        if (sb) {
+            sib.b = sb->w; sib.ldb = sb->ldw; sib.bias = sb->bias;
+            sib.c = sb->y.p[g]; sib.ldc = sb->y.ld; sib.n = sb->y.cols;
+            if (sb->st) {
+                sib.colstats = sb->st->partials[g]; sib.colstats_bytes = sb->st->bytes; sib.h_chunks = &sb->st->chunks[g];
+                call.colstats_sums = sb->st->sums;
+            }
+            call.sib = &sib;
+        }
         c.check(gemm_run(call));
     }
 }
@@ -311,6 +334,20 @@
 static bool walk_pays(int mode, int ns, int cin, int nq) {
     if (mode != 1) return mode == 2;
     return (size_t)ns * (size_t)cin * sizeof(float) > (size_t)8 << 20 && nq >= 2048;
+}
+
+static bool siblings_on(const Ctx& c, int kind) {
+    const DebugOpts& o = debug_opts();
+    return (o.siblings & kind) && gemm_split_terms_on() && !o.deterministic && o.stat_sums && !c.bf16;
+}
+static bool siblings_pay(const Ctx& c, int kind, const Mat& x, int n_first, int n_sib) {
+    if (!siblings_on(c, kind)) return false;
+    long total = 0;
+    for (int g = 0; g < c.G; ++g) {
+        if (x.rows[g] < 1) return false;
+        total += x.rows[g];
+    }
+    return gemm_x6_sibling_ok(c.max_rows(x.rows), n_first, n_sib, x.cols, total, false);
 }
 
 const int* const* level_walks(Ctx& c, const Batches& B, Walks& W, int l) {
@@ -481,7 +518,14 @@
     return true;
 }
 
-Mat resnet_block(Ctx& c, const Batches& B, Walks& W, const pcrcg_block& blk, const Mat& feats) {
+struct Hoist {
+    const float* w = nullptr;
+    int ldw = 0;
+    Mat out;
+    bool done = false;
+};
+
+Mat resnet_block(Ctx& c, const Batches& B, Walks& W, const pcrcg_block& blk, const Mat& feats, Hoist* hoist = nullptr) {
     int nq[GMAX];
     out_rows(c, B, blk, nq);
     Mat y = c.mat(nq, blk.out_dim);
@@ -490,10 +534,25 @@
     void* kp_ws[GMAX] = {};
     size_t kp_wsb[GMAX] = {};
     bool packed = false;
+    Mat s2;
+    Stat s2s;
+    bool shortcut_done = false;
     if (blk.unary1) {
         Mat t = c.gemm_out(feats.rows, blk.mid_dim, feats.cols), u = c.mat(feats.rows, blk.mid_dim);
         Stat ts = stat_buffer(c, t.rows, t.cols);
-        linear(c, feats, blk.unary1, feats.cols, nullptr, t, &ts);
+        if (!blk.strided && blk.shortcut && siblings_pay(c, 1, feats, blk.mid_dim, blk.out_dim)) {
+            s2 = c.mat(feats.rows, blk.out_dim);
+            s2s = stat_buffer(c, feats.rows, blk.out_dim);
+            Sib sb{blk.shortcut, feats.cols, nullptr, s2, &s2s};
+            linear(c, feats, blk.unary1, feats.cols, nullptr, t, t.zeroed, &ts, nullptr, nullptr, &sb);
+            shortcut_done = true;
+        } else if (blk.strided && hoist && hoist->w && siblings_pay(c, 2, feats, blk.mid_dim, hoist->out.cols)) {
+            Sib sb{hoist->w, hoist->ldw, nullptr, hoist->out, nullptr};
+            linear(c, feats, blk.unary1, feats.cols, nullptr, t, t.zeroed, &ts, nullptr, nullptr, &sb);
+            hoist->done = true;
+        } else {
+            linear(c, feats, blk.unary1, feats.cols, nullptr, t, &ts);
+        }
         if (blk.mid_dim % 4 == 0 && !(blk.kp_w_pad && blk.cin_pad > blk.mid_dim)) {
             for (int g = 0; g < c.G; ++g) {
                 kp_wsb[g] = pcrcg_kpconv_ws_bytes(feats.rows[g]);
@@ -527,9 +586,11 @@
         }
     }
     if (blk.shortcut) {
-        Mat s2 = c.gemm_out(nq, blk.out_dim, sc.cols);
-        Stat s2s = stat_buffer(c, nq, blk.out_dim);
-        linear(c, sc, blk.shortcut, sc.cols, nullptr, s2, &s2s);
+        if (!shortcut_done) {
+            s2 = c.gemm_out(nq, blk.out_dim, sc.cols);
+            s2s = stat_buffer(c, nq, blk.out_dim);
+            linear(c, sc, blk.shortcut, sc.cols, nullptr, s2, &s2s);
+        }
         norm_act(c, u2, 0.1f, y, &u2s, &s2, true, &s2s);
     } else {
         norm_act(c, u2, 0.1f, y, &u2s, &sc, false);
@@ -695,10 +756,34 @@
                 const int n = B.b[g]->n_points[l];
                 W.w[l][g] = static_cast<int*>(c.raw(sizeof(int) * (size_t)(n > 0 ? n : 1)));
             }
+    const pcrcg_block* hoist_of[PCRCG_MAX_BLOCKS] = {};
+    {
+        int pushed[PCRCG_MAX_BLOCKS], sp = 0;
+        for (int i = 0; i < mdl.n_enc; ++i)
+            if (mdl.enc_skip[i]) pushed[sp++] = i;
+        for (int j = 0; j + 1 < mdl.n_dec && sp > 0; ++j) {
+            if (mdl.dec[j].type != PCRCG_BLK_UPSAMPLE || !mdl.dec_concat[j + 1]) continue;
+            const pcrcg_block& next = mdl.dec[j + 1];
+            const int i = pushed[--sp];
+            if (next.mlp_skip && (next.type == PCRCG_BLK_UNARY || next.type == PCRCG_BLK_LAST_UNARY)) hoist_of[i] = &next;
+        }
+    }
+    std::vector<Hoist> hoists;
     for (int i = 0; i < mdl.n_enc; ++i) {
-        if (mdl.enc_skip[i]) skips.push_back(x);
         const pcrcg_block& blk = mdl.enc[i];
-        x = blk.type == PCRCG_BLK_SIMPLE ? simple_block(c, B, W, blk, x) : resnet_block(c, B, W, blk, x);
+        Hoist h;
+        if (mdl.enc_skip[i]) {
+            skips.push_back(x);
+            const pcrcg_block* next = hoist_of[i];
+            if (next && blk.type != PCRCG_BLK_SIMPLE && blk.strided && blk.unary1 && next->skip_dim == x.cols && x.ld % 4 == 0 &&
+                siblings_on(c, 2)) {
+                h.w = next->mlp_skip;
+                h.ldw = next->mlp_skip_ld;
+                h.out = c.mat(x.rows, next->out_dim, pad4(next->out_dim));
+            }
+        }
+        x = blk.type == PCRCG_BLK_SIMPLE ? simple_block(c, B, W, blk, x) : resnet_block(c, B, W, blk, x, &h);
+        if (mdl.enc_skip[i]) hoists.push_back(h);
     }
     const int gd = mdl.gnn_dim;
     int nc[GMAX] = {}, ns[GMAX] = {}, nt[GMAX] = {}, zero[GMAX] = {};
@@ -809,7 +894,11 @@
                 skips.back().ld % 4 == 0) {
                 const Mat& sk = skips.back();
                 const bool last = next->type == PCRCG_BLK_LAST_UNARY;
-                Mat tt = c.mat(trows, next->out_dim, pad4(next->out_dim));
+                const Hoist& hs = hoists.back();
+                bool early = hs.w && hs.out.cols == next->out_dim;
+                for (int g = 0; g < c.G; ++g) early = early && hs.out.rows[g] == trows[g];
+                const bool hoisted = early && hs.done;
+                Mat tt = early ? hs.out : c.mat(trows, next->out_dim, pad4(next->out_dim));
                 if (lazy && !(gemm_split_terms_on() && lazy_stats_ready(c, x, &xs))) materialise();
                 Mat z = c.gemm_out(x.rows, next->out_dim, x.cols, pad4(next->out_dim));
                 Fold up, add;
@@ -819,11 +908,13 @@
                 linear(c, x, next->mlp, next->mlp_ld, nullptr, z, z.zeroed, nullptr, nullptr, &up);
                 if (c.live()) {
                     FirstJob jobs[GMAX];
-                    for (int g = 0; g < c.G; ++g) jobs[g] = FirstJob{z.p[g], tabs[g]->idx, tt.p[g], z.rows[g], trows[g], tabs[g]->ld};
+                    for (int g = 0; g < c.G; ++g)
+                        jobs[g] = FirstJob{z.p[g], tabs[g]->idx, tt.p[g], z.rows[g], trows[g], tabs[g]->ld, hoisted ? tt.p[g] : nullptr};
                     c.check(gather_first_multi(jobs, c.G, z.cols, z.ld, tt.ld, c.st));
                 }
-                linear(c, sk, next->mlp_skip, next->mlp_skip_ld, nullptr, tt, true, nullptr, nullptr, &add);
+                if (!hoisted) linear(c, sk, next->mlp_skip, next->mlp_skip_ld, nullptr, tt, true, nullptr, nullptr, &add);
                 skips.pop_back();
+                hoists.pop_back();
                 lazy = false;
                 x = tt;
                 if (!last) {
@@ -849,7 +940,7 @@
                         c.check(pcrcg_copy2d(s.p[g], s.ld, y.p[g] + x.cols, y.ld, s.rows[g], s.cols, c.st));
                     }
                 }
-            if (concat) skips.pop_back();
+            if (concat) { skips.pop_back(); hoists.pop_back(); }
             x = y;
         } else if (blk.type == PCRCG_BLK_UNARY) {
             materialise();
diff --git a/pcrcg_amd/csrc/scan.hip b/pcrcg_amd/csrc/scan.hip
--- a/pcrcg_amd/csrc/scan.hip
+++ b/pcrcg_amd/csrc/scan.hip
@@ -206,7 +206,7 @@
     {"x6_splitk", &DebugOpts::x6_splitk}, {"x6_t1", &DebugOpts::x6_t1}, {"x6_t2", &DebugOpts::x6_t2},
     {"gemm_tile", &DebugOpts::gemm_tile}, {"gemm_splitk", &DebugOpts::gemm_splitk},
     {"gemm_split_target", &DebugOpts::gemm_split_target}, {"deterministic", &DebugOpts::deterministic},
-    {"bwd_mfma", &DebugOpts::bwd_mfma}, {"walk", &DebugOpts::walk}};
+    {"bwd_mfma", &DebugOpts::bwd_mfma}, {"walk", &DebugOpts::walk}, {"siblings", &DebugOpts::siblings}};
 std::atomic<const DebugOpts*> g_debug{nullptr};
 std::atomic<const DebugOpts*> g_debug_env{nullptr};
 std::once_flag g_debug_once;
diff --git a/pcrcg_amd/ops.py b/pcrcg_amd/ops.py
--- a/pcrcg_amd/ops.py
+++ b/pcrcg_amd/ops.py
@@ -367,6 +367,58 @@
     return out
 
 
+def gemm_sibling(a, w0, w1=None, bias0=None, bias1=None, row_scale=None, sums=None, slope=1.0, eps=1e-5,
+                 stats0=None, stats1=None):
+    import ctypes
+    L = _lib.lib()
+    count = len(a)
+    a = [_rows(x, _F32, "a")[0].contiguous() for x in a]
+    dev, k = a[0].device, a[0].shape[1]
+    w0 = _dev(w0, _F32, "w0").contiguous()
+    n0 = w0.shape[0]
+    n1 = 0
+    if w1 is not None:
+        w1 = _dev(w1, _F32, "w1").contiguous()
+        n1 = w1.shape[0]
+    m = [x.shape[0] for x in a]
+    forms = {s for s in (stats0, stats1) if s is not None}
+    if len(forms) > 1 or not forms <= {"sums", "partials"}:
+        raise RuntimeError("pcrcg_amd.gemm_sibling: stats0 / stats1 are None, 'sums' or 'partials', one form per call")
+    use_sums = "sums" in forms
+    sbytes = 0
+    if forms:
+        sbytes = 16 * max(n0, n1, 1) if use_sums else max(L.pcrcg_gemm_colstats_bytes(max(m + [1]), n) for n in (n0, max(n1, 1)))
+
+    def stat_bufs(form, n):
+        if form is None:
+            return None
+        if use_sums:
+            return [torch.zeros((2, n), dtype=torch.float64, device=dev) for _ in a]
+        return [torch.zeros(sbytes // 8, dtype=torch.float64, device=dev) for _ in a]
+
+    c0 = [torch.empty((mg, n0), dtype=_F32, device=dev) for mg in m]
+    c1 = [torch.empty((mg, n1), dtype=_F32, device=dev) for mg in m] if n1 else None
+    st0, st1 = stat_bufs(stats0, n0), stat_bufs(stats1 if n1 else None, n1)
+    if bias0 is not None:
+        bias0 = _dev(bias0, _F32, "bias0").contiguous()
+    if bias1 is not None:
+        bias1 = _dev(bias1, _F32, "bias1").contiguous()
+    if row_scale is not None:
+        row_scale = [_dev(r, _F32, "row_scale").contiguous() for r in row_scale]
+    if sums is not None:
+        sums = [_dev(s, torch.float64, "sums").contiguous() for s in sums]
+
+    def ptrs(ts):
+        return None if ts is None else (ctypes.c_void_p * count)(*[t.data_ptr() for t in ts])
+
+    chunks = (ctypes.c_int * (2 * count))()
+    _lib.check(L.pcrcg_gemm_f32_sibling(count, ptrs(a), (ctypes.c_int * count)(*m), k, k, ptrs(row_scale), ptrs(sums), float(eps),
+                                        float(slope), w0.data_ptr(), k, n0, _ptr(bias0), ptrs(c0), n0, ptrs(st0),
+                                        _ptr(w1), k, n1, _ptr(bias1), ptrs(c1), max(n1, 1), ptrs(st1), int(use_sums), sbytes,
+                                        chunks, _stream()), "pcrcg_gemm_f32_sibling")
+    return c0, c1, st0, st1, torch.tensor(list(chunks), dtype=torch.int32).view(2, count)
+
+
 def kpconv(q_pts, s_pts, idx, x, kernel_points, weights, extent):
     L = _lib.lib()
     q_pts = _dev(q_pts, _F32, "q_pts").contiguous()
@@ -702,7 +754,7 @@
     return NeighborTranspose(tq, th, deg, n_edges, d_max, nq, ns)
 
 
-def gather_first_multi(xs, idxs, outs):
+def gather_first_multi(xs, idxs, outs, addends=None):
     L = _lib.lib()
     n = len(xs)
     if not (1 <= n <= 4 and len(idxs) == n and len(outs) == n):
@@ -721,6 +773,15 @@
         raise RuntimeError("pcrcg_amd.gather_first_multi: the clouds must share width and leading dimensions")
     ptrs = lambda ts: (ctypes.c_void_p * n)(*[t.data_ptr() for t in ts])
     ints = lambda vs: (ctypes.c_int * n)(*[int(v) for v in vs])
+    if addends is not None:
+        for ad, o in zip(addends, outs):
+            _dev(ad, _F32, "addend")
+            if ad.shape != o.shape or ad.stride() != o.stride():
+                raise RuntimeError("pcrcg_amd.gather_first_multi: an addend must have its output's shape and strides")
+        _lib.check(L.pcrcg_gather_first_add_multi(ptrs(xs), ints([x.shape[0] for x in xs]), ptrs(idxs),
+                                                  ints([i.shape[0] for i in idxs]), ints(ld_idx), ptrs(addends), ptrs(outs), n, c,
+                                                  many_x[0], many_o[0], _stream()), "pcrcg_gather_first_add_multi")
+        return outs
     _lib.check(L.pcrcg_gather_first_multi(ptrs(xs), ints([x.shape[0] for x in xs]), ptrs(idxs), ints([i.shape[0] for i in idxs]),
                                           ints(ld_idx), ptrs(outs), n, c, many_x[0], many_o[0], _stream()),
                "pcrcg_gather_first_multi")
```

Measured after the change: 626.2, median of 6. About the same (+0.8%).
